# AITRICS/Medical_Tri_Modal_Pilot

Hardware: AMD Instinct MI355X
Metric: tri-modal training samples/s (fwd+bwd+AdamW step, per-GPU batch 64) (higher is better)
Workload: dtype bf16; 1 GPU; BASELINE configs[1]: vslt_img_txt tri_mbt_vsltcls, 6 layers, d_model 256, batch 64/GPU, TIE-len 1000 (N_v=1005), 224x224 CXR, 128-tok text, dropout 0.1, mbt-only-vslt 1, imgtxt-time 1; global_batch=64, parallelism=dp1

## Files before the change

### include/mtmp.h

```cpp
#ifndef MTMP_H
#define MTMP_H
#include <stdint.h>
#ifdef __cplusplus
extern "C" {
#endif

#define MTMP_F32 0
#define MTMP_BF16 1

int mtmp_abi_version(void);
const char* mtmp_last_error(void);

int mtmp_attn_fwd(int dtype, const void* q, const void* k, const void* v, void* o, const void* res, void* o_res,
                  float* lse, const int32_t* kv_len, const float* key_norms, int B, int N, int H, int ld_qkv, int ld_o,
                  float scale, void* stream);
int mtmp_attn_fwd_grouped(int dtype, int n, const void* const* q, const void* const* k, const void* const* v, void* const* o,
                          const void* const* res, void* const* o_res, float* const* lse, const int32_t* const* kv_len,
                          const int32_t* const* row_start, const float* const* key_norms, const int* N, const int* ld_qkv,
                          const int* ld_o, int B, int H, float scale, void* stream);
int mtmp_attn_bwd_grouped(int dtype, int n, const void* const* q, const void* const* k, const void* const* v,
                          const void* const* o, const void* const* d_o, const float* const* lse, const int32_t* const* kv_len,
                          const int32_t* const* row_start, void* const* dq, void* const* dk, void* const* dv,
                          float* const* delta_ws, const int* N, const int* ld_qkv, const int* ld_o, const int* ld_do,
                          const int* ld_dqkv, int B, int H, float scale, void* stream);
int mtmp_attn_cls_fwd(int dtype, const void* q, const void* k, const void* v, int ld_qkv, const void* res, int ld_res, void* o_cls,
                      void* r1_cls, float* lse, const int32_t* kv_len, const int32_t* row_start, int B, int N, int H, int cls_tok,
                      float scale, void* stream);
int mtmp_attn_cls_bwd(int dtype, const void* q, const void* k, const void* v, int ld_qkv, const void* o_cls, const void* d_o,
                      const float* lse, const int32_t* kv_len, const int32_t* row_start, void* dq, void* dk, void* dv, int ld_dqkv,
                      int B, int N, int H, int cls_tok, float scale, void* stream);
long long mtmp_key_norms_floats(long long rows, int H);
int mtmp_key_norms(int dtype, const void* k, float* out, long long rows, int H, int ld, void* stream);

int mtmp_attn_bwd(int dtype, const void* q, const void* k, const void* v, const void* o, const void* d_o,
                  const float* lse, const int32_t* kv_len, void* dq, void* dk, void* dv, float* delta_ws, int B,
                  int N, int H, int ld_qkv, int ld_o, int ld_do, int ld_dqkv, float scale, void* stream);

int mtmp_ln_gemm(int dtype, const void* x, const float* gamma, const float* beta, const void* w, const float* bias,
                 void* y, void* xn, float* stats, int M, int N, int ldx, int ldy, float eps, int relu, float drop_p,
                 unsigned seed, const unsigned* seed_dev, void* stream);

int mtmp_ln_gemm_qkv(int dtype, const void* x, const float* gamma, const float* beta, const void* w, const float* bias,
                     void* y, void* xn, float* stats, float* key_norms, int M, int ldx, float eps, void* stream);

int mtmp_gemm_nt(int dtype, const void* a, const void* w, const float* bias, const void* res, void* y, int M, int N,
                 int K, int lda, int ldy, int ldr, int act, float drop_p, unsigned seed, const unsigned* seed_dev,
                 const void* gate, float gate_scale, const float* row_scale, int rows_per_scale, void* stream);

long long mtmp_sign_bits_bytes(int M, int N);
int mtmp_ln_gemm_signs(int dtype, const void* x, const float* gamma, const float* beta, const void* w, const float* bias,
                       void* y, void* xn, float* stats, int M, int N, int ldx, int ldy, float eps, float drop_p,
                       unsigned seed, const unsigned* seed_dev, void* signs, void* stream);
int mtmp_gemm_nt_signs(int dtype, const void* a, const void* w, void* y, int M, int N, int lda, int ldy,
                       const void* signs, float gate_scale, void* stream);
int mtmp_gemm_nt_signs_drop(int dtype, const void* a, const void* w, void* y, int M, int N, int lda, int ldy,
                            const void* signs, float gate_scale, float drop_p, unsigned seed, const unsigned* seed_dev,
                            void* a_out, void* stream);

long long mtmp_gemm_tn_ws_floats(int M, int N, int K);
int mtmp_gemm_tn(int dtype, const void* dy, const void* x, float* dw, float* db, float* ws, int M, int N, int K,
                 int ldy, int ldx, void* stream);
int mtmp_gemm_tn_live(int dtype, const void* dy, const void* x, float* dw, float* db, float* ws, int M, int N, int K,
                      int ldy, int ldx, const int32_t* rows_live, void* stream);

int mtmp_dropout_bwd(int dtype, const void* g_in, void* g_out, long long n, unsigned seed, const unsigned* seed_dev,
                     float p, void* stream);

int mtmp_ln_bwd_ws_floats(int M);
int mtmp_ln_bwd(int dtype, const void* z, int ldz, const float* stats, const float* gamma, const void* dy,
                const void* d_res, int ldr, void* dz, float* dgamma_dbeta, float* ws, int M, float eps, void* stream);

int mtmp_gemm_lnbwd_ws_floats(int M);
int mtmp_gemm_lnbwd(int dtype, const void* dy, const void* wt, const void* z, int ldz, const float* stats,
                    const float* gamma, const void* d_res, int ldr, void* dz, float* dgamma_dbeta, float* ws, int M,
                    int K, int ldy, float eps, void* stream);

int mtmp_tie_embed_fwd(int dtype, const float* events, const float* params, const float* ftab, void* out, int n,
                       void* stream);
int mtmp_tie_bwd_ws_floats(int n);
int mtmp_tie_embed_bwd(int dtype, const float* events, const float* params, const void* d_out, float* grads,
                       float* ws, int n, void* stream);

int mtmp_time_embed_fwd(int dtype, const float* events, const float* params, const float* ftab, void* out, int n,
                        void* stream);
int mtmp_time_embed_bwd(int dtype, const float* events, const float* params, const void* d_out, float* grads,
                        float* ws, int n, void* stream);

int mtmp_tie_embed_packed_fwd(int dtype, const float* events, const int32_t* cu_seqlens, int B, int t_pad,
                              const float* params, const float* ftab, void* out, void* stream);
int mtmp_tie_embed_packed_bwd(int dtype, const float* events, const int32_t* cu_seqlens, int B, int t_pad,
                              const float* params, const void* d_out, float* grads, float* ws, void* stream);

int mtmp_stream_input_ws_floats(int rows);
int mtmp_stream_input_fwd(int dtype, const void* x, const float* cls, const float* gamma, const float* beta,
                          const float* pe, const float* bott, void* out, float* stats, int B, int N, int nb, float eps,
                          float p, unsigned seed, const unsigned* seed_dev, const int32_t* row_start, const int32_t* kv_len,
                          void* stream);
int mtmp_stream_input_bwd(int dtype, const void* dz, const void* x, const float* cls, const float* gamma,
                          const float* stats, void* dx, float* grads, float* ws, int B, int N, int nb, float p,
                          unsigned seed, const unsigned* seed_dev, const int32_t* row_start, const int32_t* kv_len,
                          void* stream);

int mtmp_head_ws_floats(int B);
int mtmp_head_fwd(const float* cls, const float* age, const float* gender, const void* const* params, float* out, float* ws,
                  int B, float ln_eps, float bn_eps, float momentum, int training, void* stream);
int mtmp_head_bwd(const float* d_out, const float* cls, const float* age, const float* gender, const void* const* params,
                  const float* ws_fwd, float* dcls, float* g_rows, float* dw1, float* g_feat, float* db2, float* ws_bwd, int B,
                  float ln_eps, int training, void* stream);
int mtmp_head_fwd_t(int cls_dtype, const void* cls, const float* age, const float* gender, const void* const* params, float* out,
                    float* ws, int B, float ln_eps, float bn_eps, float momentum, int training, long long* num_batches_tracked,
                    void* stream);
int mtmp_head_bwd_scatter(int cls_dtype, const float* d_out, const void* cls, const float* age, const float* gender,
                          const void* const* params, const float* ws_fwd, void* dcls, float* const* dst, float* ws_bwd, int B,
                          float ln_eps, int training, void* stream);

int mtmp_bce_logits_mean(const float* logits, const float* target, float* loss, float* dlogit, int n, void* stream);

int mtmp_timestamp(unsigned long long* slot, void* stream);

int mtmp_swin_stem_fwd(int dtype, const float* img, const float* w, const float* bias, const float* ln_w,
                       const float* ln_b, void* out, int n_img, int H, int W, void* stream);

int mtmp_layernorm_rows(int dtype, const void* x, const float* w, const float* b, void* y, long long rows, int C,
                        float eps, int merge, int H, int W, void* stream);

int mtmp_swin_ln_linear(int dtype, const void* x, const float* ln_w, const float* ln_b, const void* w, const float* bias,
                        void* y, long long M, int C, int N, float eps, void* stream);

int mtmp_swin_mlp(int dtype, const void* x, const float* ln_w, const float* ln_b, const void* w1, const float* b1,
                  const void* w2, const float* b2, const float* row_scale, int rows_per_scale, void* y, long long M, int C,
                  float eps, void* stream);

int mtmp_swin_window_attn(int dtype, const void* qkv, const void* table, void* out, int n_img, int H, int W, int C,
                          int heads, int shift, float scale, void* stream);

int mtmp_adamw_step(float* param, const float* grad, float* exp_avg, float* exp_avg_sq, void* bf16_shadow,
                    long long n, float lr, float beta1, float beta2, float eps, float weight_decay, int step,
                    float grad_scale, void* stream);

int mtmp_bottleneck_exchange_fwd(int dtype, void* z_v, void* z_i, void* z_t, int B, int n_v, int n_i, int n_t,
                                 const long long* missing, int resbottle, const float* prev, float* keep,
                                 const int32_t* row_start_v, void* stream);
int mtmp_bottleneck_exchange_bwd(int dtype, void* dz_v, void* dz_i, void* dz_t, int B, int n_v, int n_i, int n_t,
                                 const long long* missing, int resbottle, const float* d_prev_in, float* d_prev_out,
                                 const int32_t* row_start_v, void* stream);

int mtmp_ln_gemm_qkv_grouped(int dtype, int n, const void* const* x, const float* const* gamma, const float* const* beta,
                             const void* const* w, const float* const* bias, void* const* y, void* const* xn, float* const* stats,
                             float* const* key_norms, const int* M, const int* ldx, float eps, const int32_t* const* rows_live,
                             void* stream);
int mtmp_ln_gemm_signs_grouped(int dtype, int n, const void* const* x, const float* const* gamma, const float* const* beta,
                               const void* const* w, const float* const* bias, void* const* y, void* const* xn, float* const* stats,
                               void* const* signs, const int* M, int N, const int* ldx, float eps, float drop_p,
                               const unsigned* seeds, const unsigned* seed_dev, const int32_t* const* rows_live, void* stream);
int mtmp_gemm_nt_grouped(int dtype, int n, const void* const* a, const void* const* w, const float* const* bias,
                         const void* const* res, void* const* y, const int* M, int N, int K, const int* lda, const int* ldy,
                         const int* ldr, int act, float drop_p, const unsigned* seeds, const unsigned* seed_dev,
                         const int32_t* const* rows_live, void* stream);
int mtmp_gemm_nt_signs_drop_grouped(int dtype, int n, const void* const* a, const void* const* w, void* const* y, const int* M, int N,
                                    const int* lda, const void* const* signs, float gate_scale, float drop_p, const unsigned* seeds,
                                    const unsigned* seed_dev, void* const* a_out, const int32_t* const* rows_live, void* stream);
int mtmp_gemm_lnbwd_grouped(int dtype, int n, const void* const* dy, const void* const* wt, const void* const* z, const int* ldz,
                            const float* const* stats, const float* const* gamma, const void* const* d_res, const int* ldr,
                            void* const* dz, float* const* ws, const int* M, int K, const int* ldy, float eps,
                            const int32_t* const* rows_live, void* stream);
int mtmp_gemm_tn_group_plan(int n, const int* M, int N, int K, int* splits_out);
int mtmp_gemm_tn_grouped(int dtype, int n, const void* const* dy, const void* const* x, float* const* ws, const int* M, int N, int K,
                         const int* ldy, const int* ldx, const int* splits, const int32_t* const* rows_live, void* stream);

int mtmp_gemm_tn_slab_rows(int dtype, int M, int N, int K);
int mtmp_gemm_lnbwd_slab_rows(int M);
int mtmp_reduce_batch(const float* const* slab, const int* rows, const long long* cols, float* const* out_a, const long long* split,
                      float* const* out_b, int n, void* stream);

int mtmp_stream_input_slab_rows(int rows);
int mtmp_stream_input_bwd_partials(int dtype, const void* dz, const void* x, const float* cls, const float* gamma, const float* stats,
                                   void* dx, float* ws, int B, int N, int nb, float p, unsigned seed, const unsigned* seed_dev,
                                   const int32_t* row_start, const int32_t* kv_len, void* stream);
int mtmp_stream_input_bwd_grouped(int dtype, int n, const void* const* dz, const void* const* x, const float* const* cls,
                                  const float* const* gamma, const float* const* stats, void* const* dx, float* ws, const int* B,
                                  const int* N, const int* nb, const float* p, const unsigned* seed, const unsigned* seed_dev,
                                  const int32_t* const* row_start, const int32_t* const* kv_len, const void* const* add,
                                  const int* add_L, void* stream);
int mtmp_stream_input_fwd_add(int dtype, const void* x, const float* cls, const float* gamma, const float* beta, const float* pe,
                              const float* bott, void* out, float* stats, int B, int N, int nb, float eps, float p, unsigned seed,
                              const unsigned* seed_dev, const int32_t* row_start, const int32_t* kv_len, const void* add,
                              int add_L, void* stream);
int mtmp_token_sums(int dtype, int n, const void* const* dx, void* const* out, const int* rows, const int* L, void* stream);
int mtmp_tie_bwd_slab_rows(int n);
int mtmp_tie_time_embed_bwd_partials(int dtype, const float* events, int n, const float* time_events, int n_time, int n_time_a,
                                     const float* params, const void* d_out, const void* d_time_a, const void* d_time_b, float* ws,
                                     void* stream);
int mtmp_reduce_scatter(const float* const* src, const int* rows, const long long* ld, const long long* cols, float* const* out, int n,
                        void* stream);

int mtmp_publish_scalar(const float* value, unsigned* pair, void* stream);

int mtmp_copy_batch(const void* const* src, void* const* dst, const long long* bytes, const int* round16, int n, void* stream);

int mtmp_transpose_batch(int elem_bytes, const void* const* src, void* const* dst, const int* rows, const int* cols, int n,
                         void* stream);

int mtmp_stream_lengths(const long long* len_v, const long long* len_i, const long long* len_t, int* out, int B, int n_bott,
                        int txt_idx, void* stream);
int mtmp_image_slots(const long long* pattern, int present_below, int32_t* out, int B, int hw0, void* stream);
int mtmp_swin_stem_fwd_live(int dtype, const float* img, const float* w, const float* bias, const float* ln_w, const float* ln_b,
                            void* out, int n_img, int H, int W, const int32_t* order, const int32_t* rows_live, void* stream);
int mtmp_layernorm_rows_live(int dtype, const void* x, const float* w, const float* b, void* y, long long rows, int C, float eps,
                             int merge, int H, int W, const int32_t* rows_live, void* stream);
int mtmp_swin_ln_linear_live(int dtype, const void* x, const float* ln_w, const float* ln_b, const void* w, const float* bias,
                             void* y, long long M, int C, int N, float eps, const int32_t* rows_live, void* stream);
int mtmp_swin_mlp_live(int dtype, const void* x, const float* ln_w, const float* ln_b, const void* w1, const float* b1,
                       const void* w2, const float* b2, const float* row_scale, int rows_per_scale, void* y, long long M, int C,
                       float eps, const int32_t* rows_live, void* stream);
int mtmp_swin_window_attn_live(int dtype, const void* qkv, const void* table, void* out, int n_img, int H, int W, int C, int heads,
                               int shift, float scale, const int32_t* rows_live, void* stream);

int mtmp_layernorm_rows_bwd_slab_rows(long long rows, int C);
int mtmp_layernorm_rows_bwd(int dtype, const void* x, const float* w, const void* dy, void* dx, float* slab, long long rows, int C,
                            float eps, void* stream);
int mtmp_gelu_fwd(int dtype, const void* x, void* y, long long n, void* stream);
int mtmp_gelu_bwd(int dtype, const void* x, const void* dy, void* dx, long long n, void* stream);
int mtmp_swin_window_attn_bwd(int dtype, const void* qkv, const void* table, const void* dout, void* dqkv, float* dtab, int n_img,
                              int H, int W, int C, int heads, int shift, float scale, void* stream);

int mtmp_swin_attn_block(int dtype, const void* x, const float* ln_w, const float* ln_b, float eps, const void* wqkv,
                         const float* bqkv, const void* table, const void* wproj, const float* bproj, const float* row_scale,
                         void* out, int n_img, int H, int W, int C, int heads, int shift, float scale, const int32_t* rows_live,
                         void* stream);
int mtmp_gemm_nt_live(int dtype, const void* a, const void* w, const float* bias, const void* res, void* y, int M, int N, int K,
                      int lda, int ldy, int ldr, int act, float drop_p, unsigned seed, const unsigned* seed_dev, const void* gate,
                      float gate_scale, const float* row_scale, int rows_per_scale, const int32_t* rows_live, void* stream);

int mtmp_row_starts(const int32_t* kv_len, int32_t* out, int B, int n_max, void* stream);

#ifdef __cplusplus
}
#endif
#endif
```

### medical_tri_modal_pilot_amd/_lib.py

```python
import ctypes
import os
from ctypes import c_char_p, c_float, c_int, c_longlong, c_uint, c_void_p

_HERE = os.path.dirname(os.path.abspath(__file__))
LIB_PATH = os.environ.get("MTMP_LIB", os.path.join(_HERE, "libmtmp_hip.so"))

F32, BF16 = 0, 1

SIGNATURES = {
    "mtmp_abi_version": (c_int, []),
    "mtmp_last_error": (c_char_p, []),
    "mtmp_attn_fwd": (c_int, [c_int] + [c_void_p] * 9 + [c_int] * 5 + [c_float, c_void_p]),
    "mtmp_attn_cls_fwd": (c_int, [c_int] + [c_void_p] * 3 + [c_int, c_void_p, c_int] + [c_void_p] * 5 + [c_int] * 4 + [c_float, c_void_p]),
    "mtmp_attn_cls_bwd": (c_int, [c_int] + [c_void_p] * 3 + [c_int] + [c_void_p] * 8 + [c_int] * 5 + [c_float, c_void_p]),
    "mtmp_attn_fwd_grouped": (c_int, [c_int, c_int] + [c_void_p] * 13 + [c_int, c_int, c_float, c_void_p]),
    "mtmp_attn_bwd_grouped": (c_int, [c_int, c_int] + [c_void_p] * 17 + [c_int, c_int, c_float, c_void_p]),
    "mtmp_key_norms_floats": (c_longlong, [c_longlong, c_int]),
    "mtmp_key_norms": (c_int, [c_int, c_void_p, c_void_p, c_longlong, c_int, c_int, c_void_p]),
    "mtmp_attn_bwd": (c_int, [c_int] + [c_void_p] * 11 + [c_int] * 7 + [c_float, c_void_p]),
    "mtmp_ln_gemm": (c_int, [c_int] + [c_void_p] * 8 + [c_int] * 4 + [c_float, c_int, c_float, c_uint, c_void_p, c_void_p]),
    "mtmp_ln_gemm_qkv": (c_int, [c_int] + [c_void_p] * 9 + [c_int, c_int, c_float, c_void_p]),
    "mtmp_gemm_nt": (c_int, [c_int] + [c_void_p] * 5 + [c_int] * 7 + [c_float, c_uint, c_void_p, c_void_p, c_float, c_void_p, c_int,
                             c_void_p]),
    "mtmp_gemm_nt_live": (c_int, [c_int] + [c_void_p] * 5 + [c_int] * 7 + [c_float, c_uint, c_void_p, c_void_p, c_float, c_void_p, c_int,
                             c_void_p, c_void_p]),
    "mtmp_sign_bits_bytes": (c_longlong, [c_int, c_int]),
    "mtmp_ln_gemm_signs": (c_int, [c_int] + [c_void_p] * 8 + [c_int] * 4 + [c_float, c_float, c_uint, c_void_p, c_void_p, c_void_p]),
    "mtmp_gemm_nt_signs": (c_int, [c_int] + [c_void_p] * 3 + [c_int] * 4 + [c_void_p, c_float, c_void_p]),
    "mtmp_gemm_nt_signs_drop": (c_int, [c_int] + [c_void_p] * 3 + [c_int] * 4 + [c_void_p, c_float, c_float, c_uint, c_void_p,
                                                                                   c_void_p, c_void_p]),
    "mtmp_ln_gemm_qkv_grouped": (c_int, [c_int, c_int] + [c_void_p] * 11 + [c_float, c_void_p, c_void_p]),
    "mtmp_ln_gemm_signs_grouped": (c_int, [c_int, c_int] + [c_void_p] * 10 + [c_int, c_void_p, c_float, c_float, c_void_p, c_void_p,
                                                                                   c_void_p, c_void_p]),
    "mtmp_gemm_nt_grouped": (c_int, [c_int, c_int] + [c_void_p] * 6 + [c_int, c_int] + [c_void_p] * 3 + [c_int, c_float, c_void_p,
                                                                                                       c_void_p, c_void_p, c_void_p]),
    "mtmp_gemm_nt_signs_drop_grouped": (c_int, [c_int, c_int] + [c_void_p] * 4 + [c_int, c_void_p, c_void_p, c_float, c_float,
                                                                                  c_void_p, c_void_p, c_void_p, c_void_p, c_void_p]),
    "mtmp_gemm_lnbwd_grouped": (c_int, [c_int, c_int] + [c_void_p] * 11 + [c_int, c_void_p, c_float, c_void_p, c_void_p]),
    "mtmp_gemm_tn_group_plan": (c_int, [c_int, c_void_p, c_int, c_int, c_void_p]),
    "mtmp_gemm_tn_grouped": (c_int, [c_int, c_int] + [c_void_p] * 4 + [c_int, c_int] + [c_void_p] * 4 + [c_void_p]),
    "mtmp_gemm_tn_slab_rows": (c_int, [c_int] * 4),
    "mtmp_gemm_lnbwd_slab_rows": (c_int, [c_int]),
    "mtmp_reduce_batch": (c_int, [c_void_p] * 6 + [c_int, c_void_p]),
    "mtmp_reduce_scatter": (c_int, [c_void_p] * 5 + [c_int, c_void_p]),
    "mtmp_stream_input_slab_rows": (c_int, [c_int]),
    "mtmp_stream_input_bwd_partials": (c_int, [c_int] + [c_void_p] * 7 + [c_int] * 3 + [c_float, c_uint, c_void_p, c_void_p, c_void_p, c_void_p]),
    "mtmp_stream_input_bwd_grouped": (c_int, [c_int, c_int] + [c_void_p] * 18),
    "mtmp_stream_input_fwd_add": (c_int, [c_int] + [c_void_p] * 8 + [c_int] * 3 + [c_float, c_float, c_uint, c_void_p, c_void_p, c_void_p, c_void_p, c_int, c_void_p]),
    "mtmp_token_sums": (c_int, [c_int, c_int] + [c_void_p] * 5),
    "mtmp_tie_bwd_slab_rows": (c_int, [c_int]),
    "mtmp_tie_time_embed_bwd_partials": (c_int, [c_int, c_void_p, c_int, c_void_p, c_int, c_int] + [c_void_p] * 6),
    "mtmp_publish_scalar": (c_int, [c_void_p, c_void_p, c_void_p]),
    "mtmp_copy_batch": (c_int, [c_void_p] * 4 + [c_int, c_void_p]),
    "mtmp_stream_lengths": (c_int, [c_void_p] * 4 + [c_int] * 3 + [c_void_p]),
    "mtmp_row_starts": (c_int, [c_void_p, c_void_p, c_int, c_int, c_void_p]),
    "mtmp_image_slots": (c_int, [c_void_p, c_int, c_void_p, c_int, c_int, c_void_p]),
    "mtmp_transpose_batch": (c_int, [c_int, c_void_p, c_void_p, c_void_p, c_void_p, c_int, c_void_p]),
    "mtmp_layernorm_rows": (c_int, [c_int] + [c_void_p] * 4 + [c_longlong, c_int, c_float, c_int, c_int, c_int, c_void_p]),
    "mtmp_layernorm_rows_live": (c_int, [c_int] + [c_void_p] * 4 + [c_longlong, c_int, c_float, c_int, c_int, c_int, c_void_p, c_void_p]),
    "mtmp_swin_window_attn": (c_int, [c_int] + [c_void_p] * 3 + [c_int] * 6 + [c_float, c_void_p]),
    "mtmp_swin_window_attn_live": (c_int, [c_int] + [c_void_p] * 3 + [c_int] * 6 + [c_float, c_void_p, c_void_p]),
    "mtmp_layernorm_rows_bwd_slab_rows": (c_int, [c_longlong, c_int]),
    "mtmp_layernorm_rows_bwd": (c_int, [c_int] + [c_void_p] * 5 + [c_longlong, c_int, c_float, c_void_p]),
    "mtmp_gelu_fwd": (c_int, [c_int, c_void_p, c_void_p, c_longlong, c_void_p]),
    "mtmp_gelu_bwd": (c_int, [c_int, c_void_p, c_void_p, c_void_p, c_longlong, c_void_p]),
    "mtmp_swin_window_attn_bwd": (c_int, [c_int] + [c_void_p] * 5 + [c_int] * 6 + [c_float, c_void_p]),
    "mtmp_gemm_tn_ws_floats": (c_longlong, [c_int, c_int, c_int]),
    "mtmp_gemm_tn": (c_int, [c_int] + [c_void_p] * 5 + [c_int] * 5 + [c_void_p]),
    "mtmp_gemm_tn_live": (c_int, [c_int] + [c_void_p] * 5 + [c_int] * 5 + [c_void_p, c_void_p]),
    "mtmp_ln_bwd_ws_floats": (c_int, [c_int]),
    "mtmp_ln_bwd": (c_int, [c_int, c_void_p, c_int, c_void_p, c_void_p, c_void_p, c_void_p, c_int, c_void_p,
                            c_void_p, c_void_p, c_int, c_float, c_void_p]),
    "mtmp_gemm_lnbwd_ws_floats": (c_int, [c_int]),
    "mtmp_gemm_lnbwd": (c_int, [c_int, c_void_p, c_void_p, c_void_p, c_int, c_void_p, c_void_p, c_void_p, c_int, c_void_p,
                                c_void_p, c_void_p, c_int, c_int, c_int, c_float, c_void_p]),
    "mtmp_tie_embed_fwd": (c_int, [c_int] + [c_void_p] * 4 + [c_int, c_void_p]),
    "mtmp_tie_bwd_ws_floats": (c_int, [c_int]),
    "mtmp_tie_embed_bwd": (c_int, [c_int] + [c_void_p] * 5 + [c_int, c_void_p]),
    "mtmp_time_embed_fwd": (c_int, [c_int] + [c_void_p] * 4 + [c_int, c_void_p]),
    "mtmp_time_embed_bwd": (c_int, [c_int] + [c_void_p] * 5 + [c_int, c_void_p]),
    "mtmp_tie_embed_packed_fwd": (c_int, [c_int, c_void_p, c_void_p, c_int, c_int, c_void_p, c_void_p, c_void_p, c_void_p]),
    "mtmp_tie_embed_packed_bwd": (c_int, [c_int, c_void_p, c_void_p, c_int, c_int, c_void_p, c_void_p, c_void_p, c_void_p, c_void_p]),
    "mtmp_stream_input_ws_floats": (c_int, [c_int]),
    "mtmp_stream_input_fwd": (c_int, [c_int] + [c_void_p] * 8 + [c_int] * 3 + [c_float, c_float, c_uint, c_void_p, c_void_p, c_void_p, c_void_p]),
    "mtmp_stream_input_bwd": (c_int, [c_int] + [c_void_p] * 8 + [c_int] * 3 + [c_float, c_uint, c_void_p, c_void_p, c_void_p, c_void_p]),
    "mtmp_head_ws_floats": (c_int, [c_int]),
    "mtmp_head_fwd": (c_int, [c_void_p] * 6 + [c_int, c_float, c_float, c_float, c_int, c_void_p]),
    "mtmp_head_bwd": (c_int, [c_void_p] * 12 + [c_int, c_float, c_int, c_void_p]),
    "mtmp_head_fwd_t": (c_int, [c_int] + [c_void_p] * 6 + [c_int, c_float, c_float, c_float, c_int, c_void_p, c_void_p]),
    "mtmp_head_bwd_scatter": (c_int, [c_int] + [c_void_p] * 9 + [c_int, c_float, c_int, c_void_p]),
    "mtmp_bce_logits_mean": (c_int, [c_void_p] * 4 + [c_int, c_void_p]),
    "mtmp_timestamp": (c_int, [c_void_p, c_void_p]),
    "mtmp_swin_ln_linear": (c_int, [c_int] + [c_void_p] * 6 + [c_longlong, c_int, c_int, c_float, c_void_p]),
    "mtmp_swin_ln_linear_live": (c_int, [c_int] + [c_void_p] * 6 + [c_longlong, c_int, c_int, c_float, c_void_p, c_void_p]),
    "mtmp_swin_mlp": (c_int, [c_int] + [c_void_p] * 8 + [c_int, c_void_p, c_longlong, c_int, c_float, c_void_p]),
    "mtmp_swin_mlp_live": (c_int, [c_int] + [c_void_p] * 8 + [c_int, c_void_p, c_longlong, c_int, c_float, c_void_p, c_void_p]),
    "mtmp_swin_attn_block": (c_int, [c_int] + [c_void_p] * 3 + [c_float] + [c_void_p] * 7 + [c_int] * 6 + [c_float, c_void_p, c_void_p]),
    "mtmp_swin_stem_fwd": (c_int, [c_int] + [c_void_p] * 6 + [c_int] * 3 + [c_void_p]),
    "mtmp_swin_stem_fwd_live": (c_int, [c_int] + [c_void_p] * 6 + [c_int] * 3 + [c_void_p, c_void_p, c_void_p]),
    "mtmp_adamw_step": (c_int, [c_void_p] * 5 + [c_longlong] + [c_float] * 5 + [c_int, c_float, c_void_p]),
    "mtmp_bottleneck_exchange_fwd": (c_int, [c_int] + [c_void_p] * 3 + [c_int] * 4 + [c_void_p, c_int, c_void_p, c_void_p, c_void_p, c_void_p]),
    "mtmp_bottleneck_exchange_bwd": (c_int, [c_int] + [c_void_p] * 3 + [c_int] * 4 + [c_void_p, c_int, c_void_p, c_void_p, c_void_p, c_void_p]),
    "mtmp_dropout_bwd": (c_int, [c_int, c_void_p, c_void_p, c_longlong, c_uint, c_void_p, c_float, c_void_p]),
}

_lib = None


def lib():
    global _lib
    if _lib is None:
        if not os.path.exists(LIB_PATH):
            raise RuntimeError(
                f"{LIB_PATH} not found: the HIP extension is not built. Run `python -c 'import __graft_entry__ as g; "
                "g.build()'` (or `make -C medical_tri_modal_pilot_amd/csrc`). There is no CPU fallback.")
        L = ctypes.CDLL(LIB_PATH)
        for name, (res, args) in SIGNATURES.items():
            fn = getattr(L, name)
            fn.restype, fn.argtypes = res, args
        _lib = L
    return _lib


def check(rc: int, what: str = ""):
    if rc != 0:
        msg = lib().mtmp_last_error()
        raise RuntimeError(f"libmtmp_hip {what} failed (status {rc}): {msg.decode() if msg else '?'}")


def call(name: str, *args):
    check(getattr(lib(), name)(*args), name)
```

### medical_tri_modal_pilot_amd/csrc/attention.hip

```cpp
#include "common.hip.h"
#include <math.h>
#include <type_traits>

namespace {

constexpr int DH = 64;
constexpr int KT = 64;
constexpr int LDT = DH + 8;
constexpr float LOG2E = 1.4426950408889634f;

template <typename T> struct AttnArgs {
    const T* q; const T* k; const T* v;
    T* o; const T* res; T* o_res;
    float* lse; const int* kv_len;
    const float* knorm;
    int B, N, H, ld_qkv, ld_o;
    float scale;
    const int* row_start = nullptr;
};

constexpr int LDR = 96;

template <typename T> constexpr int tr_elems() { return sizeof(T) == 2 ? KT * LDR : DH * LDT; }

template <typename T> MTMP_DEV void tile_map(int tid, int& ra, int& rb, int& col) {
    if (sizeof(T) == 2) { ra = tid >> 3; rb = ra + 32; col = (tid & 7) * 8; }
    else                { ra = (tid & 31) * 2; rb = ra + 1; col = (tid >> 5) * 8; }
}
typedef short s16x4 __attribute__((ext_vector_type(4)));
MTMP_DEV Frag<bf16> frag_tr(const bf16* img, int row0, int col0, int lane) {
    const int G = lane >> 4, i = lane & 15;
    const bf16* a = img + (row0 + 8 * (G >> 1) + (i >> 2)) * LDR + col0 + 16 * (G & 1) + 4 * (i & 3);
    typedef __attribute__((address_space(3))) s16x4 lds_s16x4;
    const s16x4 lo = __builtin_amdgcn_ds_read_tr16_b64_v4i16((lds_s16x4*)a);
    const s16x4 hi = __builtin_amdgcn_ds_read_tr16_b64_v4i16((lds_s16x4*)(a + 4 * LDR));
    typedef short s16x8 __attribute__((ext_vector_type(8)));
    Frag<bf16> f;
    f.v = __builtin_bit_cast(bf16x8, s16x8{lo[0], lo[1], lo[2], lo[3], hi[0], hi[1], hi[2], hi[3]});
    return f;
}
MTMP_DEV Frag<float> frag_tr(const float* img, int row0, int col0, int lane) {
    return frag_load<float>(img + (col0 + (lane & 31)) * LDT + row0 + 8 * (lane >> 5));
}

template <typename T>
MTMP_DEV void tile_qk(f32x16& acc, const T* lds_rows, int r, int half, const Frag<T> (&bf)[4]) {
    const T* arow = lds_rows + swz23(r) * LDT + 8 * half;
    acc = mma0<T>(frag_load<T>(arow), bf[0]);
#pragma unroll
    for (int c = 1; c < 4; ++c) mma<T>(acc, frag_load<T>(arow + 16 * c), bf[c]);
}

template <typename T> struct TileR { Frag<T> a, b; };

template <typename T> MTMP_DEV void put_rows_r(T* dst, const TileR<T>& t, int tid) {
    int ra, rb, col;
    tile_map<T>(tid, ra, rb, col);
    frag_store<T>(dst + ra * LDT + col, t.a);
    frag_store<T>(dst + rb * LDT + col, t.b);
}
MTMP_DEV void put_tr_r(bf16* dst, const TileR<bf16>& t, int tid) {
    int ra, rb, col;
    tile_map<bf16>(tid, ra, rb, col);
    frag_store<bf16>(dst + ra * LDR + col, t.a);
    frag_store<bf16>(dst + rb * LDR + col, t.b);
}
MTMP_DEV void put_tr_r(float* dst, const TileR<float>& t, int tid) {
    float* d = dst + (tid >> 5) * 8 * LDT + (tid & 31) * 2;
#pragma unroll
    for (int e = 0; e < 8; ++e) *reinterpret_cast<f32x2*>(d + e * LDT) = f32x2{t.a.v[e], t.b.v[e]};
}
template <typename T> MTMP_DEV Frag<T> frag_scale(const Frag<T>& f, float s) {
    Frag<T> r;
#pragma unroll
    for (int j = 0; j < 8; ++j) r.v[j] = from_f32<T>(to_f32(f.v[j]) * s);
    return r;
}
constexpr float FAST_BOUND = 64.0f;
constexpr int FWD_QW = 64;
constexpr int FWD_QWG = 4 * FWD_QW;

template <typename T> constexpr int fwd_stage_elems() { return KT * LDT + tr_elems<T>(); }

template <typename T>
__global__ __launch_bounds__(256, (sizeof(T) == 2 ? 2 : 1)) void attn_fwd_kernel(Grouped<AttnArgs<T>> grp) {
    extern __shared__ __attribute__((aligned(16))) char smem_raw[];
    T* sbase = reinterpret_cast<T*>(smem_raw);
    const int wg = xcd_remap(blockIdx.x, gridDim.x);
    const int seg = grp_find(grp, wg);
    const AttnArgs<T>& p = grp.seg[seg];
    const int w = wg - grp.first[seg];
    const int nqt = (p.N + FWD_QWG - 1) / FWD_QWG;
    const int qt = w % nqt, bh = w / nqt, hd = bh % p.H;
    const int b = p.row_start ? p.row_start[p.B + 1 + bh / p.H] : bh / p.H;
    const int tid = threadIdx.x, lane = tid & 63, wave = tid >> 6;
    const int r = lane & 31, half = lane >> 5;
    int kvl = p.kv_len ? min(p.kv_len[b], p.N) : p.N;
    const int row0 = p.row_start ? p.row_start[b] : b * p.N;
    const int Nq = p.row_start ? max(kvl, 0) : p.N;
    if (qt * FWD_QWG >= Nq) return;
    const bool uniform = kvl <= 0;
    if (uniform) kvl = Nq;
    const size_t base = (size_t)row0 * p.ld_qkv + hd * DH;
    const T* Qb = p.q + base; const T* Kb = p.k + base; const T* Vb = p.v + base;
    const int q0w = qt * FWD_QWG + wave * FWD_QW;
    const int blk0 = row0 >> 5, blk1 = (row0 + Nq - 1) >> 5;
    float km = 0.f;
    if (p.knorm) km = p.knorm[(size_t)min(blk0 + lane, blk1) * p.H + hd];
    Frag<T> qf[2][4];
#pragma unroll
    for (int qb = 0; qb < 2; ++qb) {
        const int qrow = q0w + 32 * qb + r;
#pragma unroll
        for (int c = 0; c < 4; ++c)
            qf[qb][c] = frag_keep(frag_load<T>(Qb + (size_t)min(qrow, Nq - 1) * p.ld_qkv + 16 * c + 8 * half),
                                  qrow < Nq && !uniform);
    }
    const float c2 = p.scale * LOG2E;
    f32x16 o[2][2] = {{{0}, {0}}, {{0}, {0}}};
    float m[2] = {-INFINITY, -INFINITY}, l[2] = {0.f, 0.f};
    const int nfull = kvl / KT, ntiles = (kvl + KT - 1) / KT;
    int ra, rb, col;
    tile_map<T>(tid, ra, rb, col);
    const size_t tstep = (size_t)KT * p.ld_qkv;
    const T* kpa = Kb + (size_t)ra * p.ld_qkv + col;
    const T* kpb = Kb + (size_t)rb * p.ld_qkv + col;
    const ptrdiff_t kv_off = Vb - Kb;
    TileR<T> kreg, vreg;
    auto fetch = [&](int t) {
        if (t < nfull) {
            kreg.a = frag_load<T>(kpa); kreg.b = frag_load<T>(kpb);
            vreg.a = frag_load<T>(kpa + kv_off); vreg.b = frag_load<T>(kpb + kv_off);
            kpa += tstep; kpb += tstep;
        } else {
            const T* ka = Kb + (size_t)min(t * KT + ra, kvl - 1) * p.ld_qkv + col;
            const T* kb_ = Kb + (size_t)min(t * KT + rb, kvl - 1) * p.ld_qkv + col;
            kreg.a = frag_load<T>(ka); kreg.b = frag_load<T>(kb_);
            vreg.a = frag_load<T>(ka + kv_off); vreg.b = frag_load<T>(kb_ + kv_off);
        }
    };
    auto put = [&](int t) {
        T* sK = sbase + (t & 1) * fwd_stage_elems<T>();
        put_rows_r<T>(sK, kreg, tid);
        put_tr_r(sK + KT * LDT, vreg, tid);
    };
    fetch(0);
    bool fast = false;
    if (p.knorm) {
        float qs = 0.f;
#pragma unroll
        for (int qb = 0; qb < 2; ++qb) {
            float s = 0.f;
#pragma unroll
            for (int c = 0; c < 4; ++c)
#pragma unroll
                for (int j = 0; j < 8; ++j) s = fmaf(to_f32(qf[qb][c].v[j]), to_f32(qf[qb][c].v[j]), s);
            qs = fmaxf(qs, s);
        }
        qs = half_sum(qs) ;
        for (int i = blk0 + lane + 64; i <= blk1; i += 64) km = fmaxf(km, p.knorm[(size_t)i * p.H + hd]);
        km = wave_max(km);
        const float bound = sqrtf(qs) * km * (c2 * 1.02f);
        fast = wave_all(bound <= FAST_BOUND);
    }
    put(0);
    if (ntiles > 1) fetch(1);
    auto tile_begin = [&](int it) {
        __syncthreads();
        if (it + 1 < ntiles) put(it + 1);
        if (it + 2 < ntiles) fetch(it + 2);
    };
    auto load_k = [&](const T* sK, int kb, Frag<T> (&ka)[4]) {
        const T* arow = sK + (32 * kb + swz23(r)) * LDT + 8 * half;
#pragma unroll
        for (int c = 0; c < 4; ++c) ka[c] = frag_load<T>(arow + 16 * c);
    };
    auto load_v = [&](const T* sV, int kb, Frag<T> (&vt)[2][2]) {
#pragma unroll
        for (int s = 0; s < 2; ++s) {
            vt[s][0] = frag_tr(sV, 32 * kb + 16 * s, 0, lane);
            vt[s][1] = frag_tr(sV, 32 * kb + 16 * s, 32, lane);
        }
    };
    auto scores = [&](f32x16& st, const Frag<T> (&ka)[4], int qb) {
        st = mma0<T>(ka[0], qf[qb][0]);
#pragma unroll
        for (int c = 1; c < 4; ++c) mma<T>(st, ka[c], qf[qb][c]);
    };
    auto tail_c = [&](int k0) {
        f32x16 c;
#pragma unroll
        for (int t = 0; t < 16; ++t) c[t] = (k0 + acc_row_swz(t, half) >= kvl) ? -INFINITY : 0.f;
        return c;
    };
    auto scores_c = [&](f32x16& st, const Frag<T> (&ka)[4], int qb, const f32x16& c) {
        st = mma_c<T>(ka[0], qf[qb][0], c);
#pragma unroll
        for (int c4 = 1; c4 < 4; ++c4) mma<T>(st, ka[c4], qf[qb][c4]);
    };
    auto pv = [&](int qb, const Frag<T> (&pf)[2], const Frag<T> (&vt)[2][2]) {
#pragma unroll
        for (int s = 0; s < 2; ++s) {
            mma<T>(o[qb][0], vt[s][0], pf[s]);
            mma<T>(o[qb][1], vt[s][1], pf[s]);
        }
    };
    if (fast) {
#pragma unroll
        for (int qb = 0; qb < 2; ++qb)
#pragma unroll
            for (int c = 0; c < 4; ++c) qf[qb][c] = frag_scale<T>(qf[qb][c], c2);
        auto soft = [&](f32x16& st, int qb, Frag<T> (&pf)[2]) {
#pragma unroll
            for (int t = 0; t < 16; ++t) {
                const float e = fast_exp2(st[t]);
                l[qb] += e;
                st[t] = e;
            }
            pf[0] = frag_from_acc<T>(st, 0);
            pf[1] = frag_from_acc<T>(st, 1);
        };
        auto interleave = [&]() {
            if (sizeof(T) == 2) {
#pragma unroll
                for (int g = 0; g < 4; ++g) {
                    __builtin_amdgcn_sched_group_barrier(0x008, 1, 0);
                    __builtin_amdgcn_sched_group_barrier(0x400, 4, 0);
                }
#pragma unroll
                for (int g = 0; g < 4; ++g) {
                    __builtin_amdgcn_sched_group_barrier(0x008, 1, 0);
                    __builtin_amdgcn_sched_group_barrier(0x002, 6, 0);
                }
            }
        };
        auto body_rot = [&](int it, auto tail_tag, f32x16& s11, Frag<T> (&p01)[2], Frag<T> (&vtp)[2][2]) {
            constexpr bool TAIL = decltype(tail_tag)::value;
            __syncthreads();
            const T* sK = sbase + (it & 1) * fwd_stage_elems<T>();
            const T* sV = sK + KT * LDT;
            const int k0 = it * KT;
            f32x16 s00, s10, s01;
            Frag<T> ka0[4], ka1[4], vt0[2][2], p00[2], p10[2], p11[2];
            load_k(sK, 0, ka0);
            if (it + 1 < ntiles) put(it + 1);
            if (it + 2 < ntiles) fetch(it + 2);
            f32x16 c0, c1;
            if (TAIL) { c0 = tail_c(k0); c1 = tail_c(k0 + 32); }
            pv(0, p01, vtp);
            if (TAIL) scores_c(s00, ka0, 0, c0); else scores(s00, ka0, 0);
            soft(s11, 1, p11);
            load_v(sV, 0, vt0);
            interleave();
            __builtin_amdgcn_sched_barrier(0);
            pv(1, p11, vtp);
            if (TAIL) scores_c(s10, ka0, 1, c0); else scores(s10, ka0, 1);
            soft(s00, 0, p00);
            load_k(sK, 1, ka1);
            interleave();
            __builtin_amdgcn_sched_barrier(0);
            pv(0, p00, vt0);
            if (TAIL) scores_c(s01, ka1, 0, c1); else scores(s01, ka1, 0);
            soft(s10, 1, p10);
            load_v(sV, 1, vtp);
            interleave();
            __builtin_amdgcn_sched_barrier(0);
            pv(1, p10, vt0);
            if (TAIL) scores_c(s11, ka1, 1, c1); else scores(s11, ka1, 1);
            soft(s01, 0, p01);
            interleave();
            __builtin_amdgcn_sched_barrier(0);
        };
        {
            f32x16 s11;
            Frag<T> p01[2] = {frag_zero<T>(), frag_zero<T>()}, vtp[2][2] = {{frag_zero<T>(), frag_zero<T>()}, {frag_zero<T>(), frag_zero<T>()}};
#pragma unroll
            for (int t = 0; t < 16; ++t) s11[t] = -INFINITY;
            for (int it = 0; it < nfull; ++it) body_rot(it, std::false_type{}, s11, p01, vtp);
            if (ntiles > nfull) body_rot(nfull, std::true_type{}, s11, p01, vtp);
            Frag<T> p11[2];
            pv(0, p01, vtp);
            soft(s11, 1, p11);
            __builtin_amdgcn_sched_barrier(0);
            pv(1, p11, vtp);
        }
        m[0] = m[1] = 0.f;
    } else {
        auto body = [&](int it, auto tail_tag) {
            constexpr bool TAIL = decltype(tail_tag)::value;
            tile_begin(it);
            const T* sK = sbase + (it & 1) * fwd_stage_elems<T>();
            const T* sV = sK + KT * LDT;
#pragma unroll
            for (int kb = 0; kb < 2; ++kb) {
                Frag<T> ka[4], vt[2][2];
                load_k(sK, kb, ka);
                load_v(sV, kb, vt);
                f32x16 ct;
                if (TAIL) ct = tail_c(it * KT + 32 * kb);
#pragma unroll
                for (int qb = 0; qb < 2; ++qb) {
                    f32x16 st;
                    if (TAIL) scores_c(st, ka, qb, ct); else scores(st, ka, qb);
                    const float seed = fmaxf(st[15], st[14]);
                    float mxa = max3(seed, st[0], st[1]), mxb = max3(seed, st[2], st[3]);
#pragma unroll
                    for (int t = 4; t < 12; t += 4) {
                        mxa = max3(mxa, st[t], st[t + 1]);
                        mxb = max3(mxb, st[t + 2], st[t + 3]);
                    }
                    const float mx = half_max(max3(mxa, mxb, fmaxf(st[12], st[13]))) * c2;
                    if (!wave_all(mx <= m[qb])) {
                        const float m_new = fmaxf(m[qb], mx);
                        const float alpha = fast_exp2(m[qb] - m_new);
                        l[qb] *= alpha; o[qb][0] *= alpha; o[qb][1] *= alpha;
                        m[qb] = m_new;
                    }
#pragma unroll
                    for (int t = 0; t < 16; ++t) {
                        const float e = fast_exp2(fmaf(st[t], c2, -m[qb]));
                        l[qb] += e;
                        st[t] = e;
                    }
                    Frag<T> pf[2] = {frag_from_acc<T>(st, 0), frag_from_acc<T>(st, 1)};
                    pv(qb, pf, vt);
                }
            }
        };
        for (int it = 0; it < nfull; ++it) body(it, std::false_type{});
        if (ntiles > nfull) body(nfull, std::true_type{});
    }
    constexpr int E = 16 / (int)sizeof(T);
    constexpr int CH = DH * (int)sizeof(T) / 16, RPP = 64 / CH, NPS = FWD_QW / RPP;
    const int rsub = lane / CH, ch = lane % CH;
    u32x4_t rv[NPS];
    if (p.o_res) {
#pragma unroll
        for (int ps = 0; ps < NPS; ++ps) {
            const int rowc = min(q0w + ps * RPP + rsub, Nq - 1);
            rv[ps] = *reinterpret_cast<const u32x4_t*>(p.res + ((size_t)row0 + rowc) * p.ld_o + hd * DH + ch * E);
        }
    }
    __syncthreads();
    T* sO = reinterpret_cast<T*>(smem_raw) + wave * FWD_QW * LDT;
#pragma unroll
    for (int qb = 0; qb < 2; ++qb) {
        l[qb] = half_sum(l[qb]);
        const float inv = 1.0f / l[qb];
#pragma unroll
        for (int dt = 0; dt < 2; ++dt)
#pragma unroll
            for (int g = 0; g < 4; ++g) {
                const f32x16& ov = o[qb][dt];
                store4<T>(sO + (32 * qb + r) * LDT + 32 * dt + 8 * g + 4 * half, ov[4 * g] * inv, ov[4 * g + 1] * inv,
                          ov[4 * g + 2] * inv, ov[4 * g + 3] * inv);
            }
        const int qrow = q0w + 32 * qb + r;
        if (qrow < Nq && half == 0) p.lse[((size_t)b * p.H + hd) * p.N + qrow] = m[qb] + log2f(l[qb]);
    }
    asm volatile("s_waitcnt lgkmcnt(0)" ::: "memory");
    u32x4_t ovv[NPS];
#pragma unroll
    for (int ps = 0; ps < NPS; ++ps)
        ovv[ps] = *reinterpret_cast<const u32x4_t*>(reinterpret_cast<const char*>(sO + (ps * RPP + rsub) * LDT) + 16 * ch);
    T* orow = p.o + ((size_t)row0 + q0w + rsub) * p.ld_o + hd * DH + ch * E;
#pragma unroll
    for (int ps = 0; ps < NPS; ++ps)
        if (q0w + ps * RPP + rsub < Nq) *reinterpret_cast<u32x4_t*>(orow + (size_t)ps * RPP * p.ld_o) = ovv[ps];
    if (p.o_res) {
        T* rrow = p.o_res + ((size_t)row0 + q0w + rsub) * p.ld_o + hd * DH + ch * E;
#pragma unroll
        for (int ps = 0; ps < NPS; ++ps) {
            T ob[E], rbv[E], sb[E];
            __builtin_memcpy(ob, &ovv[ps], 16);
            __builtin_memcpy(rbv, &rv[ps], 16);
#pragma unroll
            for (int i = 0; i < E; ++i) sb[i] = from_f32<T>(to_f32(ob[i]) + to_f32(rbv[i]));
            u32x4_t sv;
            __builtin_memcpy(&sv, sb, 16);
            if (q0w + ps * RPP + rsub < Nq) *reinterpret_cast<u32x4_t*>(rrow + (size_t)ps * RPP * p.ld_o) = sv;
        }
    }
}

template <typename T> __global__ __launch_bounds__(256) void key_norms_kernel(const T* k, float* out, int M, int H, int ld) {
    const int lane = threadIdx.x & 63, blk = blockIdx.x * 4 + (threadIdx.x >> 6);
    if (blk * 32 >= M) return;
    const int rsub = lane >> 3, ch = lane & 7;
    for (int h = 0; h < H; ++h) {
        float best = 0.f;
#pragma unroll
        for (int ps = 0; ps < 4; ++ps) {
            const int row = min(blk * 32 + ps * 8 + rsub, M - 1);
            const Frag<T> f = frag_load<T>(k + (size_t)row * ld + h * DH + 8 * ch);
            float s = 0.f;
#pragma unroll
            for (int j = 0; j < 8; ++j) s = fmaf(to_f32(f.v[j]), to_f32(f.v[j]), s);
            s += __shfl_xor(s, 1, 64); s += __shfl_xor(s, 2, 64); s += __shfl_xor(s, 4, 64);
            best = fmaxf(best, s);
        }
        best = fmaxf(best, __shfl_xor(best, 8, 64));
        best = fmaxf(best, __shfl_xor(best, 16, 64));
        best = fmaxf(best, __shfl_xor(best, 32, 64));
        if (lane == 0) out[(size_t)blk * H + h] = sqrtf(best);
    }
}



template <typename T> struct DualTile;
template <> struct DualTile<bf16> {
    static constexpr int BYTES = 8192;
    static MTMP_DEV void map(int tid, int& ra, int& rb, int& ca, int& cb) { ra = rb = tid >> 2; ca = 8 * (tid & 3); cb = 32 + 8 * (tid & 3); }
    static MTMP_DEV int off(int row, int ch) {
        return 1024 * (row >> 3) + 512 * (ch >> 2) + 64 * (row & 7) + 16 * ((ch & 3) ^ ((row >> 2) & 3));
    }
    static MTMP_DEV void put(char* img, const TileR<bf16>& t, int tid) {
        const int row = tid >> 2, c = tid & 3;
        *reinterpret_cast<bf16x8*>(img + off(row, c)) = t.a.v;
        *reinterpret_cast<bf16x8*>(img + off(row, 4 + c)) = t.b.v;
    }
    static MTMP_DEV Frag<bf16> row_frag(const char* img, int row, int c, int half) {
        Frag<bf16> f;
        f.v = *reinterpret_cast<const bf16x8*>(img + off(row, 2 * c + half));
        return f;
    }
    static MTMP_DEV Frag<bf16> tr_frag(const char* img, int row0, int col0, int lane) {
        const int G = lane >> 4, i = lane & 15;
        const int row = row0 + 8 * (G >> 1) + (i >> 2), col = col0 + 16 * (G & 1) + 4 * (i & 3);
        typedef __attribute__((address_space(3))) s16x4 lds_s16x4;
        const s16x4 lo = __builtin_amdgcn_ds_read_tr16_b64_v4i16((lds_s16x4*)(img + off(row, col >> 3) + 2 * (col & 7)));
        const s16x4 hi = __builtin_amdgcn_ds_read_tr16_b64_v4i16((lds_s16x4*)(img + off(row + 4, col >> 3) + 2 * (col & 7)));
        typedef short s16x8 __attribute__((ext_vector_type(8)));
        Frag<bf16> f;
        f.v = __builtin_bit_cast(bf16x8, s16x8{lo[0], lo[1], lo[2], lo[3], hi[0], hi[1], hi[2], hi[3]});
        return f;
    }
};
template <> struct DualTile<float> {
    static constexpr int BYTES = (KT * LDT + DH * LDT) * 4;
    static MTMP_DEV void map(int tid, int& ra, int& rb, int& ca, int& cb) { ra = (tid & 31) * 2; rb = ra + 1; ca = cb = (tid >> 5) * 8; }
    static MTMP_DEV void put(char* img, const TileR<float>& t, int tid) {
        float* rows = reinterpret_cast<float*>(img);
        put_rows_r<float>(rows, t, tid);
        put_tr_r(rows + KT * LDT, t, tid);
    }
    static MTMP_DEV Frag<float> row_frag(const char* img, int row, int c, int half) {
        return frag_load<float>(reinterpret_cast<const float*>(img) + row * LDT + 16 * c + 8 * half);
    }
    static MTMP_DEV Frag<float> tr_frag(const char* img, int row0, int col0, int lane) {
        return frag_tr(reinterpret_cast<const float*>(img) + KT * LDT, row0, col0, lane);
    }
};

template <typename T> struct TileStream {
    const T* base; const T* pa; const T* pb;
    size_t step; int ld, limit, ra, rb, ca, cb, nfull;
    MTMP_DEV void init(const T* src, int ld_, int limit_, int tid) {
        DualTile<T>::map(tid, ra, rb, ca, cb);
        base = src; ld = ld_; limit = limit_; nfull = limit_ / KT; step = (size_t)KT * ld_;
        pa = src + (size_t)ra * ld_ + ca; pb = src + (size_t)rb * ld_ + cb;
    }
    MTMP_DEV TileR<T> fetch(int t) {
        TileR<T> x;
        if (t < nfull) {
            x.a = frag_load<T>(pa); x.b = frag_load<T>(pb);
            pa += step; pb += step;
        } else {
            x.a = frag_load<T>(base + (size_t)min(t * KT + ra, limit - 1) * ld + ca);
            x.b = frag_load<T>(base + (size_t)min(t * KT + rb, limit - 1) * ld + cb);
        }
        return x;
    }
    MTMP_DEV TileR<T> zero_tail(const TileR<T>& x, int t) const {
        TileR<T> y;
        y.a = frag_keep(x.a, t * KT + ra < limit);
        y.b = frag_keep(x.b, t * KT + rb < limit);
        return y;
    }
};
template <typename T> struct AttnBwdArgs {
    const T* q; const T* k; const T* v; const T* d_o;
    const float* lse; float* delta; const int* kv_len;
    T* dq; T* dk; T* dv;
    int B, N, H, ld_qkv, ld_do, ld_dqkv;
    float scale;
    const T* o; int ld_o;
    const int* row_start = nullptr;
};


template <typename T> constexpr int dq_stage_bytes() { return 2 * DualTile<T>::BYTES; }
template <typename T>
__global__ __launch_bounds__(256, (sizeof(T) == 2 ? 2 : 1)) void attn_bwd_dq_kernel(Grouped<AttnBwdArgs<T>> grp) {
    using DT = DualTile<T>;
    extern __shared__ __attribute__((aligned(16))) char smem_raw[];
    const int wg = xcd_remap(blockIdx.x, gridDim.x);
    const int seg = grp_find(grp, wg);
    const AttnBwdArgs<T>& p = grp.seg[seg];
    const int w = wg - grp.first[seg];
    const int nqt = (p.N + 127) >> 7;
    const int qt = w % nqt, bh = w / nqt, hd = bh % p.H;
    const int b = p.row_start ? p.row_start[p.B + 1 + bh / p.H] : bh / p.H;
    const int tid = threadIdx.x, lane = tid & 63, wave = tid >> 6;
    const int r = lane & 31, half = lane >> 5;
    int kvl = p.kv_len ? min(p.kv_len[b], p.N) : p.N;
    const int row0 = p.row_start ? p.row_start[b] : b * p.N;
    const int Nq = p.row_start ? max(kvl, 0) : p.N;
    if (qt * 128 >= Nq) return;
    const bool uniform = kvl <= 0;
    if (uniform) kvl = Nq;
    const size_t base = (size_t)row0 * p.ld_qkv + hd * DH;
    const T* Qb = p.q + base; const T* Kb = p.k + base; const T* Vb = p.v + base;
    const int qrow = qt * 128 + wave * 32 + r;
    const float c2 = p.scale * LOG2E;
    const size_t sidx = ((size_t)b * p.H + hd) * p.N + min(qrow, Nq - 1);
    const float lse_v = p.lse[sidx];
    Frag<T> qf[4], dof[4], of[4];
#pragma unroll
    for (int c = 0; c < 4; ++c) {
        qf[c] = frag_load<T>(Qb + (size_t)min(qrow, Nq - 1) * p.ld_qkv + 16 * c + 8 * half);
        dof[c] = frag_load<T>(p.d_o + ((size_t)row0 + min(qrow, Nq - 1)) * p.ld_do + hd * DH + 16 * c + 8 * half);
        of[c] = frag_load<T>(p.o + ((size_t)row0 + min(qrow, Nq - 1)) * p.ld_o + hd * DH + 16 * c + 8 * half);
    }
    const int ntiles = uniform ? 0 : (kvl + KT - 1) / KT;
    const int nfull = kvl / KT;
    TileStream<T> ks, vs;
    ks.init(Kb, p.ld_qkv, kvl, tid);
    vs.init(Vb, p.ld_qkv, kvl, tid);
    TileR<T> kreg, vreg;
    auto fetch = [&](int t) { kreg = ks.fetch(t); vreg = vs.fetch(t); };
    auto put = [&](int t) {
        char* st_ = smem_raw + (t & 1) * dq_stage_bytes<T>();
        DT::put(st_, t >= nfull ? ks.zero_tail(kreg, t) : kreg, tid);
        DT::put(st_ + DT::BYTES, vreg, tid);
    };
    if (ntiles > 0) fetch(0);
#pragma unroll
    for (int c = 0; c < 4; ++c) {
        qf[c] = frag_keep(frag_scale<T>(qf[c], c2), qrow < Nq);
        dof[c] = frag_keep(dof[c], qrow < Nq);
    }
    float dsum = 0.f;
#pragma unroll
    for (int c = 0; c < 4; ++c)
#pragma unroll
        for (int jx = 0; jx < 8; ++jx) dsum = fmaf(to_f32(dof[c].v[jx]), to_f32(of[c].v[jx]), dsum);
    dsum = half_sum(dsum);
    if (qrow < Nq && half == 0) p.delta[sidx] = dsum;
    const float nL = (qrow < Nq) ? -lse_v : -INFINITY;
    const float nD = (qrow < Nq) ? -dsum : 0.f;
    f32x16 cL, cD;
#pragma unroll
    for (int t = 0; t < 16; ++t) { cL[t] = nL; cD[t] = nD; }
    f32x16 dq0 = {0}, dq1 = {0};
    if (ntiles > 0) put(0);
    if (ntiles > 1) fetch(1);
    struct Unit { f32x16 st, dp; };
    auto body = [&](int it, auto tail_tag) {
        constexpr bool TAIL = decltype(tail_tag)::value;
        const int k0 = it * KT;
        __syncthreads();
        const char* sK = smem_raw + (it & 1) * dq_stage_bytes<T>();
        const char* sV = sK + DT::BYTES;
        auto load_rows = [&](int kb, Frag<T> (&ka)[4], Frag<T> (&va)[4]) {
            const int row = 32 * kb + swz23(r);
#pragma unroll
            for (int c = 0; c < 4; ++c) { ka[c] = DT::row_frag(sK, row, c, half); va[c] = DT::row_frag(sV, row, c, half); }
        };
        auto load_tr = [&](int kb, Frag<T> (&trf)[2][2]) {
#pragma unroll
            for (int s = 0; s < 2; ++s) {
                trf[s][0] = DT::tr_frag(sK, 32 * kb + 16 * s, 0, lane);
                trf[s][1] = DT::tr_frag(sK, 32 * kb + 16 * s, 32, lane);
            }
        };
        auto scores = [&](int kb, Unit& u, const Frag<T> (&ka)[4], const Frag<T> (&va)[4]) {
            if (TAIL) {
                f32x16 cLt;
#pragma unroll
                for (int t = 0; t < 16; ++t) cLt[t] = (k0 + 32 * kb + acc_row_swz(t, half) < kvl) ? nL : -INFINITY;
                u.st = mma_c<T>(ka[0], qf[0], cLt);
            } else
            u.st = mma_c<T>(ka[0], qf[0], cL);
#pragma unroll
            for (int c = 1; c < 4; ++c) mma<T>(u.st, ka[c], qf[c]);
            u.dp = mma_c<T>(va[0], dof[0], cD);
#pragma unroll
            for (int c = 1; c < 4; ++c) mma<T>(u.dp, va[c], dof[c]);
        };
        auto soft = [&](Unit& u, Frag<T> (&dsf)[2]) {
#pragma unroll
            for (int t = 0; t < 16; ++t) u.st[t] = fast_exp2(u.st[t]) * u.dp[t];
            dsf[0] = frag_from_acc<T>(u.st, 0);
            dsf[1] = frag_from_acc<T>(u.st, 1);
        };
        auto grad = [&](const Frag<T> (&dsf)[2], const Frag<T> (&trf)[2][2]) {
#pragma unroll
            for (int s = 0; s < 2; ++s) {
                mma<T>(dq0, trf[s][0], dsf[s]);
                mma<T>(dq1, trf[s][1], dsf[s]);
            }
        };
        Unit u0, u1;
        Frag<T> d0[2], d1[2], ka0[4], va0[4], ka1[4], va1[4], tr0[2][2], tr1[2][2];
        load_rows(0, ka0, va0);
        if (it + 1 < ntiles) put(it + 1);
        if (it + 2 < ntiles) fetch(it + 2);
        __builtin_amdgcn_sched_barrier(0);
        load_rows(1, ka1, va1);
        scores(0, u0, ka0, va0);
        if (sizeof(T) == 2) {
#pragma unroll
            for (int g = 0; g < 8; ++g) {
                __builtin_amdgcn_sched_group_barrier(0x008, 1, 0);
                __builtin_amdgcn_sched_group_barrier(0x100, 1, 0);
            }
        }
        __builtin_amdgcn_sched_barrier(0);
        load_tr(0, tr0);
        scores(1, u1, ka1, va1);
        soft(u0, d0);
        if (sizeof(T) == 2) {
#pragma unroll
            for (int g = 0; g < 8; ++g) {
                __builtin_amdgcn_sched_group_barrier(0x008, 1, 0);
                __builtin_amdgcn_sched_group_barrier(0x100, 1, 0);
                __builtin_amdgcn_sched_group_barrier(0x400, 2, 0);
                __builtin_amdgcn_sched_group_barrier(0x002, 3, 0);
            }
        }
        __builtin_amdgcn_sched_barrier(0);
        load_tr(1, tr1);
        grad(d0, tr0);
        soft(u1, d1);
        if (sizeof(T) == 2) {
#pragma unroll
            for (int g = 0; g < 4; ++g) {
                __builtin_amdgcn_sched_group_barrier(0x008, 1, 0);
                __builtin_amdgcn_sched_group_barrier(0x100, 2, 0);
                __builtin_amdgcn_sched_group_barrier(0x400, 4, 0);
                __builtin_amdgcn_sched_group_barrier(0x002, 6, 0);
            }
        }
        __builtin_amdgcn_sched_barrier(0);
        grad(d1, tr1);
    };
    for (int it = 0; it < min(nfull, ntiles); ++it) body(it, std::false_type{});
    if (ntiles > nfull) body(nfull, std::true_type{});
    if (qrow < Nq) {
        const size_t orow = ((size_t)row0 + qrow) * p.ld_dqkv + hd * DH;
#pragma unroll
        for (int dt = 0; dt < 2; ++dt)
#pragma unroll
            for (int g = 0; g < 4; ++g) {
                const f32x16& o = dt ? dq1 : dq0;
                const int d0 = 32 * dt + 8 * g + 4 * half;
                store4<T>(p.dq + orow + d0, o[4 * g] * p.scale, o[4 * g + 1] * p.scale, o[4 * g + 2] * p.scale,
                          o[4 * g + 3] * p.scale);
            }
    }
}

template <typename T> constexpr int dkdv_stage_bytes() { return 2 * DualTile<T>::BYTES + 2 * KT * (int)sizeof(float); }
template <typename T>
__global__ __launch_bounds__(256, (sizeof(T) == 2 ? 2 : 1)) void attn_bwd_dkdv_kernel(Grouped<AttnBwdArgs<T>> grp) {
    using DT = DualTile<T>;
    extern __shared__ __attribute__((aligned(16))) char smem_raw[];
    const int wg = xcd_remap(blockIdx.x, gridDim.x);
    const int seg = grp_find(grp, wg);
    const AttnBwdArgs<T>& p = grp.seg[seg];
    const int w = wg - grp.first[seg];
    const int nkt = (p.N + 127) >> 7;
    const int kt = w % nkt, bh = w / nkt, hd = bh % p.H;
    const int b = p.row_start ? p.row_start[p.B + 1 + bh / p.H] : bh / p.H;
    const int tid = threadIdx.x, lane = tid & 63, wave = tid >> 6;
    const int r = lane & 31, half = lane >> 5;
    int kvl = p.kv_len ? min(p.kv_len[b], p.N) : p.N;
    const int row0 = p.row_start ? p.row_start[b] : b * p.N;
    const int Nq = p.row_start ? max(kvl, 0) : p.N;
    if (kt * 128 >= Nq) return;
    const bool uniform = kvl <= 0;
    if (uniform) kvl = Nq;
    const size_t base = (size_t)row0 * p.ld_qkv + hd * DH;
    const T* Qb = p.q + base; const T* Kb = p.k + base; const T* Vb = p.v + base;
    const T* dOb = p.d_o + (size_t)row0 * p.ld_do + hd * DH;
    const float* Lb = p.lse + ((size_t)b * p.H + hd) * p.N;
    const float* Db = p.delta + ((size_t)b * p.H + hd) * p.N;
    const int kw0 = kt * 128 + wave * 32;
    const int key = kw0 + r;
    f32x16 dk0 = {0}, dk1 = {0}, dv0 = {0}, dv1 = {0};
    if (kt * 128 < kvl) {
        const float c2 = p.scale * LOG2E;
        Frag<T> kf[4], vf[4];
#pragma unroll
        for (int c = 0; c < 4; ++c) {
            kf[c] = frag_keep(frag_scale<T>(frag_load<T>(Kb + (size_t)min(key, kvl - 1) * p.ld_qkv + 16 * c + 8 * half), c2),
                              key < kvl && !uniform);
            vf[c] = frag_keep(frag_load<T>(Vb + (size_t)min(key, kvl - 1) * p.ld_qkv + 16 * c + 8 * half), key < kvl);
        }
        const int nq = (Nq + KT - 1) / KT;
        TileStream<T> qs, os;
        qs.init(Qb, p.ld_qkv, Nq, tid);
        os.init(dOb, p.ld_do, Nq, tid);
        TileR<T> qreg, oreg;
        const int lrow = tid & (KT - 1);
        float lreg, dreg;
        auto fetch = [&](int t) {
            qreg = qs.fetch(t);
            oreg = os.fetch(t);
            const int qn = min(t * KT + lrow, Nq - 1);
            lreg = Lb[qn];
            dreg = Db[qn];
        };
        auto put = [&](int t) {
            char* st_ = smem_raw + (t & 1) * dkdv_stage_bytes<T>();
            DT::put(st_, qreg, tid);
            DT::put(st_ + DT::BYTES, oreg, tid);
            if (tid < KT) {
                float* sL = reinterpret_cast<float*>(st_ + 2 * DT::BYTES);
                sL[tid] = (t * KT + tid < Nq) ? -lreg : -INFINITY;
                sL[KT + tid] = (t * KT + tid < Nq) ? -dreg : 0.f;
            }
        };
        fetch(0);
        put(0);
        if (nq > 1) fetch(1);
        for (int it = 0; it < nq; ++it) {
            __syncthreads();
            if (it + 1 < nq) put(it + 1);
            if (it + 2 < nq) fetch(it + 2);
            if (kw0 < kvl) {
                const char* sQ = smem_raw + (it & 1) * dkdv_stage_bytes<T>();
                const char* sdO = sQ + DT::BYTES;
                const float* sL = reinterpret_cast<const float*>(sQ + 2 * DT::BYTES);
                const float* sD = sL + KT;
                auto load_rowconst = [&](int qb, f32x16& cL, f32x16& cD) {
#pragma unroll
                    for (int h8 = 0; h8 < 2; ++h8)
#pragma unroll
                        for (int v = 0; v < 2; ++v) {
                            const f32x4 l4 = *reinterpret_cast<const f32x4*>(sL + 32 * qb + 16 * h8 + 8 * half + 4 * v);
                            const f32x4 d4 = *reinterpret_cast<const f32x4*>(sD + 32 * qb + 16 * h8 + 8 * half + 4 * v);
#pragma unroll
                            for (int i = 0; i < 4; ++i) { cL[8 * h8 + 4 * v + i] = l4[i]; cD[8 * h8 + 4 * v + i] = d4[i]; }
                        }
                };
                auto load_rows = [&](int qb, Frag<T> (&qa)[4], Frag<T> (&oa)[4]) {
                    const int row = 32 * qb + swz23(r);
#pragma unroll
                    for (int c = 0; c < 4; ++c) { qa[c] = DT::row_frag(sQ, row, c, half); oa[c] = DT::row_frag(sdO, row, c, half); }
                };
                auto load_tr = [&](int qb, Frag<T> (&trf)[2][4]) {
#pragma unroll
                    for (int s = 0; s < 2; ++s) {
                        const int q16 = 32 * qb + 16 * s;
                        trf[s][0] = DT::tr_frag(sdO, q16, 0, lane);
                        trf[s][1] = DT::tr_frag(sdO, q16, 32, lane);
                        trf[s][2] = DT::tr_frag(sQ, q16, 0, lane);
                        trf[s][3] = DT::tr_frag(sQ, q16, 32, lane);
                    }
                };
                auto scores = [&](f32x16& st, f32x16& ds, const f32x16& cL, const f32x16& cD, const Frag<T> (&qa)[4],
                                  const Frag<T> (&oa)[4]) {
                    st = mma_c<T>(qa[0], kf[0], cL);
#pragma unroll
                    for (int c = 1; c < 4; ++c) mma<T>(st, qa[c], kf[c]);
                    ds = mma_c<T>(oa[0], vf[0], cD);
#pragma unroll
                    for (int c = 1; c < 4; ++c) mma<T>(ds, oa[c], vf[c]);
                };
                auto probs = [&](f32x16& st, f32x16& ds, Frag<T> (&pf)[2], Frag<T> (&dsf)[2]) {
#pragma unroll
                    for (int t = 0; t < 16; ++t) {
                        const float pv = fast_exp2(st[t]);
                        st[t] = pv;
                        ds[t] *= pv;
                    }
#pragma unroll
                    for (int s = 0; s < 2; ++s) { pf[s] = frag_from_acc<T>(st, s); dsf[s] = frag_from_acc<T>(ds, s); }
                };
                auto grads = [&](const Frag<T> (&pf)[2], const Frag<T> (&dsf)[2], const Frag<T> (&trf)[2][4]) {
#pragma unroll
                    for (int s = 0; s < 2; ++s) {
                        mma<T>(dv0, trf[s][0], pf[s]);
                        mma<T>(dv1, trf[s][1], pf[s]);
                        mma<T>(dk0, trf[s][2], dsf[s]);
                        mma<T>(dk1, trf[s][3], dsf[s]);
                    }
                };
                f32x16 st0, ds0, st1, ds1, cL1, cD1;
                Frag<T> qa1[4], oa1[4], pf0[2], dsf0[2], pf1[2], dsf1[2];
                {
                    f32x16 cL0, cD0;
                    Frag<T> qa0[4], oa0[4];
                    load_rowconst(0, cL0, cD0);
                    load_rows(0, qa0, oa0);
                    load_rowconst(1, cL1, cD1);
                    load_rows(1, qa1, oa1);
                    scores(st0, ds0, cL0, cD0, qa0, oa0);
                }
                __builtin_amdgcn_sched_barrier(0);
                {
                    scores(st1, ds1, cL1, cD1, qa1, oa1);
                    probs(st0, ds0, pf0, dsf0);
                    if (sizeof(T) == 2) {
#pragma unroll
                        for (int g = 0; g < 8; ++g) {
                            __builtin_amdgcn_sched_group_barrier(0x008, 1, 0);
                            __builtin_amdgcn_sched_group_barrier(0x400, 2, 0);
                            __builtin_amdgcn_sched_group_barrier(0x002, 4, 0);
                        }
                    }
                }
                __builtin_amdgcn_sched_barrier(0);
                {
                    Frag<T> trf0[2][4];
                    load_tr(0, trf0);
                    grads(pf0, dsf0, trf0);
                    probs(st1, ds1, pf1, dsf1);
                    if (sizeof(T) == 2) {
                        __builtin_amdgcn_sched_group_barrier(0x100, 16, 0);
                        __builtin_amdgcn_sched_group_barrier(0x400, 4, 0);
                        __builtin_amdgcn_sched_group_barrier(0x002, 8, 0);
#pragma unroll
                        for (int g = 0; g < 8; ++g) {
                            __builtin_amdgcn_sched_group_barrier(0x008, 1, 0);
                            if (g < 6) __builtin_amdgcn_sched_group_barrier(0x400, 2, 0);
                            if (g < 6) __builtin_amdgcn_sched_group_barrier(0x002, 4, 0);
                        }
                    }
                }
                __builtin_amdgcn_sched_barrier(0);
                {
                    Frag<T> trf1[2][4];
                    load_tr(1, trf1);
                    grads(pf1, dsf1, trf1);
                }
            }
        }
    }
    if (key < Nq) {
        const bool live = key < kvl;
        const float ks = (live && !uniform) ? p.scale : 0.f, vs_ = live ? 1.f : 0.f;
        const size_t orow = ((size_t)row0 + key) * p.ld_dqkv + hd * DH;
#pragma unroll
        for (int dt = 0; dt < 2; ++dt)
#pragma unroll
            for (int g = 0; g < 4; ++g) {
                const f32x16& ak = dt ? dk1 : dk0;
                const f32x16& av = dt ? dv1 : dv0;
                const int d0 = 32 * dt + 8 * g + 4 * half;
                store4<T>(p.dk + orow + d0, ks != 0.f ? ak[4 * g] * ks : 0.f, ks != 0.f ? ak[4 * g + 1] * ks : 0.f,
                          ks != 0.f ? ak[4 * g + 2] * ks : 0.f, ks != 0.f ? ak[4 * g + 3] * ks : 0.f);
                store4<T>(p.dv + orow + d0, vs_ != 0.f ? av[4 * g] : 0.f, vs_ != 0.f ? av[4 * g + 1] : 0.f,
                          vs_ != 0.f ? av[4 * g + 2] : 0.f, vs_ != 0.f ? av[4 * g + 3] : 0.f);
            }
    }
}

#define MTMP_MFMA_FIRST(d, a, b, c) asm volatile("v_mfma_f32_32x32x16_bf16 %0, %1, %2, %3" : "=&v"(d) : "v"(a), "a"(b), "v"(c))
#define MTMP_MFMA_NEXT(d, a, b) asm volatile("v_mfma_f32_32x32x16_bf16 %0, %1, %2, %0" : "+v"(d) : "v"(a), "a"(b))
#define MTMP_MFMA_ACC(acc, a, b) asm volatile("v_mfma_f32_32x32x16_bf16 %0, %1, %2, %0" : "+a"(acc) : "v"(a), "v"(b))

#ifdef MTMP_LAB_CLOCK
__device__ long long mtmp_dbg_stamps[64 * 4 * 160];
#define STAMP(k) do { if (wg < 64 && lane == 0 && (k) < 160) mtmp_dbg_stamps[(wg * 4 + wave) * 160 + (k)] = __builtin_amdgcn_s_memtime(); } while (0)
#else
#define STAMP(k) do {} while (0)
#endif
constexpr int DKV64_KEYS = 256;
constexpr int BWD64_MIN_ROWS = 1536;
constexpr int BWD64_STAGES = 3;
constexpr int DKV64_OUT_BYTES = 2 * 64 * LDT * 2;

MTMP_DEV bf16x8 to_agpr(bf16x8 x) {
    bf16x8 y;
    asm volatile("" : "=a"(y) : "0"(x));
    return y;
}
struct PackedUnit { u32x4_t p[2], d[2]; };
MTMP_DEV unsigned cvt_pk_bf16(float lo, float hi) {
    return __builtin_bit_cast(unsigned, __builtin_convertvector(f32x2{lo, hi}, bf16x2));
}

__global__ __launch_bounds__(256, 1) void attn_bwd_dkdv64_kernel(Grouped<AttnBwdArgs<bf16>> grp) {
    using T = bf16;
    using DT = DualTile<T>;
    extern __shared__ __attribute__((aligned(16))) char smem_raw[];
    const int wg = xcd_remap(blockIdx.x, gridDim.x);
    const int seg = grp_find(grp, wg);
    const AttnBwdArgs<T>& p = grp.seg[seg];
    const int w = wg - grp.first[seg];
    const int nkt = (p.N + DKV64_KEYS - 1) / DKV64_KEYS;
    const int kt = w % nkt, bh = w / nkt, hd = bh % p.H;
    const int b = p.row_start ? p.row_start[p.B + 1 + bh / p.H] : bh / p.H;
    const int tid = threadIdx.x, lane = tid & 63, wave = tid >> 6;
    const int r = lane & 31, half = lane >> 5;
    int kvl = p.kv_len ? min(p.kv_len[b], p.N) : p.N;
    const int row0 = p.row_start ? p.row_start[b] : b * p.N;
    const int Nq = p.row_start ? max(kvl, 0) : p.N;
    if (kt * DKV64_KEYS >= Nq) return;
    STAMP(0);
    const bool uniform = kvl <= 0;
    if (uniform) kvl = Nq;
    const size_t base = (size_t)row0 * p.ld_qkv + hd * DH;
    const T* Qb = p.q + base; const T* Kb = p.k + base; const T* Vb = p.v + base;
    const T* dOb = p.d_o + (size_t)row0 * p.ld_do + hd * DH;
    const float* Lb = p.lse + ((size_t)b * p.H + hd) * p.N;
    const float* Db = p.delta + ((size_t)b * p.H + hd) * p.N;
    const int kw0 = kt * DKV64_KEYS + wave * 64;
    f32x16 dv00 = {0}, dv01 = {0}, dk00 = {0}, dk01 = {0}, dv10 = {0}, dv11 = {0}, dk10 = {0}, dk11 = {0};
    if (kt * DKV64_KEYS < kvl) {
        const float c2 = p.scale * LOG2E;
        Frag<T> kx[2][4], vx[2][4];
#pragma unroll
        for (int kb = 0; kb < 2; ++kb)
#pragma unroll
            for (int c = 0; c < 4; ++c) {
                const int key = kw0 + 32 * kb + r;
                kx[kb][c] = frag_load<T>(Kb + (size_t)min(key, kvl - 1) * p.ld_qkv + 16 * c + 8 * half);
                vx[kb][c] = frag_load<T>(Vb + (size_t)min(key, kvl - 1) * p.ld_qkv + 16 * c + 8 * half);
            }
        const int nq = (Nq + KT - 1) / KT;
        TileStream<T> qs, os;
        qs.init(Qb, p.ld_qkv, Nq, tid);
        os.init(dOb, p.ld_do, Nq, tid);
        TileR<T> qreg, oreg;
        const int lrow = tid & (KT - 1);
        float lreg, dreg;
        auto stage = [&](int t) { return smem_raw + (t % BWD64_STAGES) * dkdv_stage_bytes<T>(); };
        auto stage_piece = [&](int k, int tp, int tf) {
            if (k < 3) {
                if (tp >= nq) return;
                char* st_ = stage(tp);
                if (k == 0) DT::put(st_, qreg, tid);
                else if (k == 1) DT::put(st_ + DT::BYTES, oreg, tid);
                else if (tid < KT) {
                    float* sL = reinterpret_cast<float*>(st_ + 2 * DT::BYTES);
                    sL[tid] = (tp * KT + tid < Nq) ? -lreg : -INFINITY;
                    sL[KT + tid] = (tp * KT + tid < Nq) ? -dreg : 0.f;
                }
            } else {
                if (tf >= nq) return;
                if (k == 3) qreg = qs.fetch(tf);
                else if (k == 4) oreg = os.fetch(tf);
                else {
                    const int qn = min(tf * KT + lrow, Nq - 1);
                    lreg = Lb[qn];
                    dreg = Db[qn];
                }
            }
        };
        auto stage_all = [&](int tp, int tf) {
#pragma unroll
            for (int k = 0; k < 6; ++k) stage_piece(k, tp, tf);
        };
        stage_all(nq, 0);
        bf16x8 kf[2][4], vf[2][4];
#pragma unroll
        for (int kb = 0; kb < 2; ++kb)
#pragma unroll
            for (int c = 0; c < 4; ++c) {
                const bool live = kw0 + 32 * kb + r < kvl;
                kf[kb][c] = to_agpr(frag_keep(frag_scale<T>(kx[kb][c], c2), live && !uniform).v);
                vf[kb][c] = to_agpr(frag_keep(vx[kb][c], live).v);
            }
        stage_all(0, 1);
        __syncthreads();
        const bool active = kw0 < kvl;
        bf16x8 qa[4], oa[4], tr[2][4];
        f32x16 cL, cD;
        struct LaneOffs { unsigned rowE, rowO, cst, trA, trB; };
        LaneOffs lo;
        {
            const int sr = swz23(r), G = lane >> 4, i16 = lane & 15;
            lo.rowE = DT::off(sr, half);
            lo.rowO = DT::off(sr, 2 + half);
            lo.cst = 2 * DT::BYTES + 32 * half;
            const int trow = 8 * (G >> 1) + (i16 >> 2), tch = 2 * (G & 1) + ((i16 & 3) >> 1);
            lo.trA = DT::off(trow, tch) + 8 * (i16 & 1);
            lo.trB = DT::off(trow + 4, tch) + 8 * (i16 & 1);
            const unsigned lds0 = (unsigned)(size_t)(__attribute__((address_space(3))) char*)smem_raw;
            lo.rowE += lds0; lo.rowO += lds0; lo.cst += lds0; lo.trA += lds0; lo.trB += lds0;
        }
        typedef __attribute__((address_space(3))) const char lds_cchar;
        auto lds_at = [](unsigned ofs) { return (lds_cchar*)(size_t)ofs; };
        auto bases = [&](int t) {
            const unsigned sb = (unsigned)((t % BWD64_STAGES) * dkdv_stage_bytes<T>());
            LaneOffs x{lo.rowE + sb, lo.rowO + sb, lo.cst + sb, lo.trA + sb, lo.trB + sb};
            asm volatile("" : "+v"(x.rowE), "+v"(x.rowO), "+v"(x.cst), "+v"(x.trA), "+v"(x.trB));
            return x;
        };
        auto load_rows = [&](const LaneOffs& bs, int qb, int c, bool dO) {
            typedef __attribute__((address_space(3))) const bf16x8 lds_bf16x8;
            const bf16x8 v = *(lds_bf16x8*)(lds_at((c & 1) ? bs.rowO : bs.rowE) + 512 * (c >> 1) + 4096 * qb + (dO ? DT::BYTES : 0));
            if (dO) oa[c] = v; else qa[c] = v;
        };
        auto load_const = [&](const LaneOffs& bs, int qb, int k4, bool dlt) {
            typedef __attribute__((address_space(3))) const f32x4 lds_f32x4;
            const f32x4 v4 = *(lds_f32x4*)(lds_at(bs.cst) + (dlt ? 4 * KT : 0) + 4 * (32 * qb + 16 * (k4 >> 1) + 4 * (k4 & 1)));
#pragma unroll
            for (int i = 0; i < 4; ++i) { if (dlt) cD[4 * k4 + i] = v4[i]; else cL[4 * k4 + i] = v4[i]; }
        };
        auto load_tr = [&](const LaneOffs& bs, int qb, int s2, int j) {
            typedef __attribute__((address_space(3))) s16x4 lds_s16x4;
            const int imm = 4096 * qb + 2048 * s2 + 512 * (j & 1) + (j < 2 ? DT::BYTES : 0);
            const s16x4 a = __builtin_amdgcn_ds_read_tr16_b64_v4i16((lds_s16x4*)(lds_at(bs.trA) + imm));
            const s16x4 b4 = __builtin_amdgcn_ds_read_tr16_b64_v4i16((lds_s16x4*)(lds_at(bs.trB) + imm));
            typedef short s16x8 __attribute__((ext_vector_type(8)));
            tr[s2][j] = __builtin_bit_cast(bf16x8, s16x8{a[0], a[1], a[2], a[3], b4[0], b4[1], b4[2], b4[3]});
        };
        auto slot = [&](auto mode_tag, f32x16& sN, f32x16& dN, const bf16x8 (&kfb)[4], const bf16x8 (&vfb)[4], f32x16& sC, f32x16& dC,
                        PackedUnit& out, const PackedUnit& in, f32x16& dv0, f32x16& dv1, f32x16& dk0, f32x16& dk1,
                        const LaneOffs& st_rows, int qb_rows, const LaneOffs& st_tr, int qb_tr, int tp, int tf) {
            constexpr int MODE = decltype(mode_tag)::value;
#pragma unroll
            for (int i = 0; i < 16; ++i) {
                if (i == 0) MTMP_MFMA_FIRST(sN, qa[0], kfb[0], cL);
                else if (i < 4) MTMP_MFMA_NEXT(sN, qa[i], kfb[i]);
                else if (i == 4) MTMP_MFMA_FIRST(dN, oa[0], vfb[0], cD);
                else if (i < 8) MTMP_MFMA_NEXT(dN, oa[i - 4], vfb[i - 4]);
                else {
                    const int s2 = (i - 8) >> 2, j = (i - 8) & 3;
                    if (j == 0) MTMP_MFMA_ACC(dv0, tr[s2][0], in.p[s2]);
                    else if (j == 1) MTMP_MFMA_ACC(dv1, tr[s2][1], in.p[s2]);
                    else if (j == 2) MTMP_MFMA_ACC(dk0, tr[s2][2], in.d[s2]);
                    else MTMP_MFMA_ACC(dk1, tr[s2][3], in.d[s2]);
                }
                const float e = fast_exp2(sC[i]);
                if (i > 0) dC[i - 1] *= sC[i - 1];
                sC[i] = e;
                if (i & 1) out.p[i >> 3][(i & 7) >> 1] = cvt_pk_bf16(sC[i - 1], e);
                if (i >= 2 && !(i & 1)) out.d[(i - 2) >> 3][((i - 2) & 7) >> 1] = cvt_pk_bf16(dC[i - 2], dC[i - 1]);
                if (i == 15) {
                    dC[15] *= e;
                    out.d[1][3] = cvt_pk_bf16(dC[14], dC[15]);
                }
                if (MODE == 1) {
                    if (i < 4) load_rows(st_rows, qb_rows, i, false);
                    else if (i < 8) load_rows(st_rows, qb_rows, i - 4, true);
                    else load_tr(st_tr, qb_tr, (i - 8) >> 2, (i - 8) & 3);
                    if (i >= 1 && i < 5) load_const(st_rows, qb_rows, i - 1, false);
                    else if (i >= 5 && i < 9) load_const(st_rows, qb_rows, i - 5, true);
                }
                if (MODE == 2 && (i & 1) && i < 12) stage_piece(i >> 1, tp, tf);
                __builtin_amdgcn_sched_barrier(0);
            }
        };
        f32x16 sA, dA, sB, dB;
        PackedUnit fX, fY;
#pragma unroll
        for (int t = 0; t < 16; ++t) { sB[t] = -INFINITY; dB[t] = 0.f; }
#pragma unroll
        for (int s2 = 0; s2 < 2; ++s2) {
            fX.p[s2] = u32x4_t{0, 0, 0, 0}; fX.d[s2] = u32x4_t{0, 0, 0, 0};
#pragma unroll
            for (int j = 0; j < 4; ++j) tr[s2][j] = frag_zero<T>().v;
        }
        if (active) {
            const LaneOffs b0 = bases(0);
#pragma unroll
            for (int c = 0; c < 4; ++c) {
                load_rows(b0, 0, c, false); load_rows(b0, 0, c, true);
                load_const(b0, 0, c, false); load_const(b0, 0, c, true);
            }
        }
        const std::integral_constant<int, 0> plain{};
        const std::integral_constant<int, 1> loads{};
        const std::integral_constant<int, 2> staging{};
        STAMP(1);
        for (int it = 0; it < nq; ++it) {
            STAMP(2 + 8 * it);
            const LaneOffs cur = bases(it);
            const LaneOffs nxt = bases(it + 1 < nq ? it + 1 : it);
            if (active) {
                __builtin_amdgcn_sched_barrier(0);
                STAMP(3 + 8 * it);
                slot(staging, sA, dA, kf[0], vf[0], sB, dB, fY, fX, dv00, dv01, dk00, dk01, cur, 0, cur, 0, it + 1, it + 2);
                STAMP(4 + 8 * it);
                slot(loads, sB, dB, kf[1], vf[1], sA, dA, fX, fY, dv10, dv11, dk10, dk11, cur, 1, cur, 0, 0, 0);
                STAMP(5 + 8 * it);
                slot(plain, sA, dA, kf[0], vf[0], sB, dB, fY, fX, dv00, dv01, dk00, dk01, cur, 0, cur, 0, 0, 0);
                STAMP(6 + 8 * it);
            } else {
                stage_all(it + 1, it + 2);
            }
            __syncthreads();
            if (active) {
                STAMP(7 + 8 * it);
                slot(loads, sB, dB, kf[1], vf[1], sA, dA, fX, fY, dv10, dv11, dk10, dk11, nxt, 0, cur, 1, 0, 0);
                STAMP(8 + 8 * it);
            }
        }
        if (active) {
#pragma unroll
            for (int i = 0; i < 16; ++i) {
                if (i < 8) {
                    const int s2 = i >> 2, j = i & 3;
                    if (j == 0) MTMP_MFMA_ACC(dv00, tr[s2][0], fX.p[s2]);
                    else if (j == 1) MTMP_MFMA_ACC(dv01, tr[s2][1], fX.p[s2]);
                    else if (j == 2) MTMP_MFMA_ACC(dk00, tr[s2][2], fX.d[s2]);
                    else MTMP_MFMA_ACC(dk01, tr[s2][3], fX.d[s2]);
                }
                const float e = fast_exp2(sB[i]);
                dB[i] *= e;
                sB[i] = e;
                if (i & 1) {
                    fY.p[i >> 3][(i & 7) >> 1] = cvt_pk_bf16(sB[i - 1], e);
                    fY.d[i >> 3][(i & 7) >> 1] = cvt_pk_bf16(dB[i - 1], dB[i]);
                }
                __builtin_amdgcn_sched_barrier(0);
            }
#pragma unroll
            for (int s2 = 0; s2 < 2; ++s2) {
                MTMP_MFMA_ACC(dv10, tr[s2][0], fY.p[s2]);
                MTMP_MFMA_ACC(dv11, tr[s2][1], fY.p[s2]);
                MTMP_MFMA_ACC(dk10, tr[s2][2], fY.d[s2]);
                MTMP_MFMA_ACC(dk11, tr[s2][3], fY.d[s2]);
            }
        }
        STAMP(150);
        asm volatile("s_nop 15\n\ts_nop 15" : "+a"(dv00), "+a"(dv01), "+a"(dk00), "+a"(dk01), "+a"(dv10), "+a"(dv11), "+a"(dk10), "+a"(dk11));
    }
    T* sOut = reinterpret_cast<T*>(smem_raw + BWD64_STAGES * dkdv_stage_bytes<T>() + wave * DKV64_OUT_BYTES);
#pragma unroll
    for (int kb = 0; kb < 2; ++kb) {
        const int key = kw0 + 32 * kb + r;
        const bool live = key < kvl;
        const bool wk = live && !uniform;
#pragma unroll
        for (int dt = 0; dt < 2; ++dt)
#pragma unroll
            for (int g = 0; g < 4; ++g) {
                const f32x16& ak = kb ? (dt ? dk11 : dk10) : (dt ? dk01 : dk00);
                const f32x16& av = kb ? (dt ? dv11 : dv10) : (dt ? dv01 : dv00);
                const int d0 = 32 * dt + 8 * g + 4 * half;
                store4<T>(sOut + (32 * kb + r) * LDT + d0, wk ? ak[4 * g] * p.scale : 0.f, wk ? ak[4 * g + 1] * p.scale : 0.f,
                          wk ? ak[4 * g + 2] * p.scale : 0.f, wk ? ak[4 * g + 3] * p.scale : 0.f);
                store4<T>(sOut + (64 + 32 * kb + r) * LDT + d0, live ? av[4 * g] : 0.f, live ? av[4 * g + 1] : 0.f,
                          live ? av[4 * g + 2] : 0.f, live ? av[4 * g + 3] : 0.f);
            }
    }
    asm volatile("s_waitcnt lgkmcnt(0)" ::: "memory");
    {
        const int rsub = lane >> 3, ch = lane & 7;
        u32x4_t ok[8], ov[8];
#pragma unroll
        for (int ps = 0; ps < 8; ++ps) {
            ok[ps] = *reinterpret_cast<const u32x4_t*>(reinterpret_cast<const char*>(sOut + (8 * ps + rsub) * LDT) + 16 * ch);
            ov[ps] = *reinterpret_cast<const u32x4_t*>(reinterpret_cast<const char*>(sOut + (64 + 8 * ps + rsub) * LDT) + 16 * ch);
        }
        T* krow = p.dk + ((size_t)row0 + kw0 + rsub) * p.ld_dqkv + hd * DH + 8 * ch;
        T* vrow = p.dv + ((size_t)row0 + kw0 + rsub) * p.ld_dqkv + hd * DH + 8 * ch;
#pragma unroll
        for (int ps = 0; ps < 8; ++ps)
            if (kw0 + 8 * ps + rsub < Nq) {
                *reinterpret_cast<u32x4_t*>(krow + (size_t)8 * ps * p.ld_dqkv) = ok[ps];
                *reinterpret_cast<u32x4_t*>(vrow + (size_t)8 * ps * p.ld_dqkv) = ov[ps];
            }
    }
    STAMP(151);
}

template <typename T> size_t fwd_smem() { return (size_t)2 * fwd_stage_elems<T>() * sizeof(T); }
template <typename T> size_t dq_smem() { return (size_t)2 * dq_stage_bytes<T>(); }
template <typename T> size_t dkdv_smem() { return (size_t)2 * dkdv_stage_bytes<T>(); }

template <typename K> int set_smem(K kern, size_t bytes) {
    if (bytes > 48 * 1024) {
        if (hipFuncSetAttribute(reinterpret_cast<const void*>(kern), hipFuncAttributeMaxDynamicSharedMemorySize,
                                (int)bytes) != hipSuccess) {
            mtmp_set_error("hipFuncSetAttribute(MaxDynamicSharedMemorySize=%zu) failed", bytes);
            return MTMP_ERR_LAUNCH;
        }
    }
    return MTMP_OK;
}

template <typename A, typename F> Grouped<A> make_group(int n, const A* segs, F blocks_of, int& total) {
    Grouped<A> g;
    total = 0;
    for (int i = 0; i < GRP_MAX; ++i) {
        g.seg[i] = segs[i < n ? i : 0];
        g.first[i] = total;
        if (i < n) total += blocks_of(segs[i]);
    }
    g.first[GRP_MAX] = total;
    return g;
}

template <typename T> int launch_fwd(int n, const AttnArgs<T>* segs, hipStream_t st) {
    int nwg;
    const Grouped<AttnArgs<T>> g = make_group(n, segs, [](const AttnArgs<T>& a) { return ((a.N + FWD_QWG - 1) / FWD_QWG) * a.H * a.B; }, nwg);
    const size_t sm = fwd_smem<T>();
    if (int e = set_smem(attn_fwd_kernel<T>, sm)) return e;
    hipLaunchKernelGGL(attn_fwd_kernel<T>, dim3(nwg), dim3(256), sm, st, g);
    MTMP_CHECK_LAUNCH("mtmp_attn_fwd");
    return MTMP_OK;
}

template <typename T> int launch_bwd(int n, const AttnBwdArgs<T>* segs, hipStream_t st) {
    int nwg;
    const Grouped<AttnBwdArgs<T>> g = make_group(n, segs, [](const AttnBwdArgs<T>& a) { return ((a.N + 127) / 128) * a.H * a.B; }, nwg);
    if (int e = set_smem(attn_bwd_dq_kernel<T>, dq_smem<T>())) return e;
    hipLaunchKernelGGL(attn_bwd_dq_kernel<T>, dim3(nwg), dim3(256), dq_smem<T>(), st, g);
    MTMP_CHECK_LAUNCH("mtmp_attn_bwd(dq)");
    if constexpr (sizeof(T) == 2) {
        int nmax = 0;
        for (int i = 0; i < n; ++i) nmax = segs[i].N > nmax ? segs[i].N : nmax;
        if (nmax >= BWD64_MIN_ROWS) {
            int nwg64;
            const Grouped<AttnBwdArgs<T>> g64 =
                make_group(n, segs, [](const AttnBwdArgs<T>& a) { return ((a.N + DKV64_KEYS - 1) / DKV64_KEYS) * a.H * a.B; }, nwg64);
            const size_t sm64 = (size_t)BWD64_STAGES * dkdv_stage_bytes<T>() + 4 * DKV64_OUT_BYTES;
            if (int e = set_smem(attn_bwd_dkdv64_kernel, sm64)) return e;
            hipLaunchKernelGGL(attn_bwd_dkdv64_kernel, dim3(nwg64), dim3(256), sm64, st, g64);
            MTMP_CHECK_LAUNCH("mtmp_attn_bwd(dkdv64)");
            return MTMP_OK;
        }
    }
    if (int e = set_smem(attn_bwd_dkdv_kernel<T>, dkdv_smem<T>())) return e;
    hipLaunchKernelGGL(attn_bwd_dkdv_kernel<T>, dim3(nwg), dim3(256), dkdv_smem<T>(), st, g);
    MTMP_CHECK_LAUNCH("mtmp_attn_bwd(dkdv)");
    return MTMP_OK;
}

bool attn_shape_ok(int B, int N, int H, int ld_a, int ld_b) {
    return B > 0 && N > 0 && H > 0 && H <= 4 && ld_a >= H * DH && ld_b >= H * DH && (ld_a % 8) == 0 && (ld_b % 8) == 0;
}

}

template <typename T>
int fwd_entry(int n, const void* const* q, const void* const* k, const void* const* v, void* const* o, const void* const* res,
              void* const* o_res, float* const* lse, const int32_t* const* kv_len, const int32_t* const* row_start,
              const float* const* key_norms, const int* N, const int* ld_qkv, const int* ld_o, int B, int H, float scale,
              hipStream_t st) {
    AttnArgs<T> a[GRP_MAX];
    for (int i = 0; i < n; ++i)
        a[i] = AttnArgs<T>{(const T*)q[i], (const T*)k[i], (const T*)v[i], (T*)o[i], res ? (const T*)res[i] : nullptr,
                           o_res ? (T*)o_res[i] : nullptr, lse[i], kv_len ? kv_len[i] : nullptr, key_norms ? key_norms[i] : nullptr,
                           B, N[i], H, ld_qkv[i], ld_o[i], scale, row_start ? row_start[i] : nullptr};
    return launch_fwd<T>(n, a, st);
}

extern "C" int mtmp_attn_fwd_grouped(int dtype, int n, const void* const* q, const void* const* k, const void* const* v,
                                     void* const* o, const void* const* res, void* const* o_res, float* const* lse,
                                     const int32_t* const* kv_len, const int32_t* const* row_start, const float* const* key_norms,
                                     const int* N, const int* ld_qkv, const int* ld_o, int B, int H, float scale, void* stream) {
    MTMP_CHECK_ARG(n >= 1 && n <= GRP_MAX && q && k && v && o && lse && N && ld_qkv && ld_o, "mtmp_attn_fwd: bad group (n=%d)", n);
    for (int i = 0; i < n; ++i) {
        MTMP_CHECK_ARG(q[i] && k[i] && v[i] && o[i] && lse[i], "mtmp_attn_fwd: null pointer (stream %d)", i);
        MTMP_CHECK_ARG((!res || !res[i]) == (!o_res || !o_res[i]), "mtmp_attn_fwd: res and o_res must be given together");
        MTMP_CHECK_ARG(!(row_start && row_start[i]) || (kv_len && kv_len[i]), "mtmp_attn_fwd: a packed stream needs kv_len");
        MTMP_CHECK_ARG(attn_shape_ok(B, N[i], H, ld_qkv[i], ld_o[i]), "mtmp_attn_fwd: bad shape B=%d N=%d H=%d ld=%d/%d", B, N[i], H,
                       ld_qkv[i], ld_o[i]);
    }
    hipStream_t st = (hipStream_t)stream;
    if (dtype == 0) return fwd_entry<float>(n, q, k, v, o, res, o_res, lse, kv_len, row_start, key_norms, N, ld_qkv, ld_o, B, H, scale, st);
    if (dtype == 1) return fwd_entry<bf16>(n, q, k, v, o, res, o_res, lse, kv_len, row_start, key_norms, N, ld_qkv, ld_o, B, H, scale, st);
    mtmp_set_error("mtmp_attn_fwd: unknown dtype %d", dtype);
    return MTMP_ERR_ARG;
}

extern "C" int mtmp_attn_fwd(int dtype, const void* q, const void* k, const void* v, void* o, const void* res,
                             void* o_res, float* lse, const int32_t* kv_len, const float* key_norms, int B, int N, int H,
                             int ld_qkv, int ld_o, float scale, void* stream) {
    return mtmp_attn_fwd_grouped(dtype, 1, &q, &k, &v, &o, &res, &o_res, &lse, &kv_len, nullptr, &key_norms, &N, &ld_qkv, &ld_o, B, H,
                                 scale, stream);
}

template <typename T>
int bwd_entry(int n, const void* const* q, const void* const* k, const void* const* v, const void* const* o, const void* const* d_o,
              const float* const* lse, const int32_t* const* kv_len, const int32_t* const* row_start, void* const* dq,
              void* const* dk, void* const* dv, float* const* delta_ws, const int* N, const int* ld_qkv, const int* ld_o,
              const int* ld_do, const int* ld_dqkv, int B, int H, float scale, hipStream_t st) {
    AttnBwdArgs<T> a[GRP_MAX];
    for (int i = 0; i < n; ++i)
        a[i] = AttnBwdArgs<T>{(const T*)q[i], (const T*)k[i], (const T*)v[i], (const T*)d_o[i], lse[i], delta_ws[i],
                              kv_len ? kv_len[i] : nullptr, (T*)dq[i], (T*)dk[i], (T*)dv[i], B, N[i], H, ld_qkv[i], ld_do[i],
                              ld_dqkv[i], scale, (const T*)o[i], ld_o[i], row_start ? row_start[i] : nullptr};
    return launch_bwd<T>(n, a, st);
}

extern "C" int mtmp_attn_bwd_grouped(int dtype, int n, const void* const* q, const void* const* k, const void* const* v,
                                     const void* const* o, const void* const* d_o, const float* const* lse,
                                     const int32_t* const* kv_len, const int32_t* const* row_start, void* const* dq,
                                     void* const* dk, void* const* dv, float* const* delta_ws, const int* N, const int* ld_qkv,
                                     const int* ld_o, const int* ld_do, const int* ld_dqkv, int B, int H, float scale, void* stream) {
    MTMP_CHECK_ARG(n >= 1 && n <= GRP_MAX && q && k && v && o && d_o && lse && dq && dk && dv && delta_ws && N && ld_qkv && ld_o &&
                       ld_do && ld_dqkv, "mtmp_attn_bwd: bad group (n=%d)", n);
    for (int i = 0; i < n; ++i) {
        MTMP_CHECK_ARG(q[i] && k[i] && v[i] && o[i] && d_o[i] && lse[i] && dq[i] && dk[i] && dv[i] && delta_ws[i],
                       "mtmp_attn_bwd: null pointer (stream %d)", i);
        MTMP_CHECK_ARG(!(row_start && row_start[i]) || (kv_len && kv_len[i]), "mtmp_attn_bwd: a packed stream needs kv_len");
        MTMP_CHECK_ARG(attn_shape_ok(B, N[i], H, ld_qkv[i], ld_o[i]) && attn_shape_ok(B, N[i], H, ld_do[i], ld_dqkv[i]),
                       "mtmp_attn_bwd: bad shape B=%d N=%d H=%d", B, N[i], H);
    }
    hipStream_t st = (hipStream_t)stream;
    if (dtype == 0)
        return bwd_entry<float>(n, q, k, v, o, d_o, lse, kv_len, row_start, dq, dk, dv, delta_ws, N, ld_qkv, ld_o, ld_do, ld_dqkv, B, H, scale, st);
    if (dtype == 1)
        return bwd_entry<bf16>(n, q, k, v, o, d_o, lse, kv_len, row_start, dq, dk, dv, delta_ws, N, ld_qkv, ld_o, ld_do, ld_dqkv, B, H, scale, st);
    mtmp_set_error("mtmp_attn_bwd: unknown dtype %d", dtype);
    return MTMP_ERR_ARG;
}

extern "C" int mtmp_attn_bwd(int dtype, const void* q, const void* k, const void* v, const void* o, const void* d_o,
                             const float* lse, const int32_t* kv_len, void* dq, void* dk, void* dv, float* delta_ws,
                             int B, int N, int H, int ld_qkv, int ld_o, int ld_do, int ld_dqkv, float scale,
                             void* stream) {
    return mtmp_attn_bwd_grouped(dtype, 1, &q, &k, &v, &o, &d_o, &lse, &kv_len, nullptr, &dq, &dk, &dv, &delta_ws, &N, &ld_qkv, &ld_o,
                                 &ld_do, &ld_dqkv, B, H, scale, stream);
}

namespace {
template <typename T> struct AttnClsArgs {
    const T* q; const T* k; const T* v; int ld_qkv;
    const T* res; int ld_res;
    T* o_cls; T* r1_cls; float* lse;
    const T* d_o;
    T* dq; T* dk; T* dv; int ld_dqkv;
    const int* kv_len; const int* row_start;
    int B, N, H, cls_tok;
    float scale;
};

template <typename T> MTMP_DEV void load8f(const T* ptr, float (&o)[8]) {
    const f32x4 a = load4<T>(ptr), b = load4<T>(ptr + 4);
    o[0] = a[0]; o[1] = a[1]; o[2] = a[2]; o[3] = a[3]; o[4] = b[0]; o[5] = b[1]; o[6] = b[2]; o[7] = b[3];
}
MTMP_DEV float block_reduce(float v, float* red, bool take_max) {
    v = take_max ? wave_max(v) : wave_sum(v);
    __syncthreads();
    if ((threadIdx.x & 63) == 0) red[threadIdx.x >> 6] = v;
    __syncthreads();
    return take_max ? fmaxf(fmaxf(red[0], red[1]), fmaxf(red[2], red[3])) : (red[0] + red[1]) + (red[2] + red[3]);
}

template <typename T> __global__ __launch_bounds__(256) void attn_cls_fwd_kernel(AttnClsArgs<T> p) {
    extern __shared__ float cls_lds[];
    float* s = cls_lds;
    float* red = s + p.N;
    float* part = red + 4;
    const int b = blockIdx.x / p.H, hd = blockIdx.x % p.H, tid = threadIdx.x;
    const int kv_raw = p.kv_len ? p.kv_len[b] : p.N;
    if (p.row_start && kv_raw <= p.cls_tok) {
        if (tid < DH) {
            const size_t oi = ((size_t)b * p.H + hd) * DH + tid;
            p.o_cls[oi] = from_f32<T>(0.f);
            p.r1_cls[oi] = from_f32<T>(0.f);
            if (tid == 0) p.lse[b * p.H + hd] = 0.f;
        }
        return;
    }
    const bool uniform = kv_raw <= 0;
    const int kvl = uniform ? p.N : min(kv_raw, p.N);
    const size_t row0 = p.row_start ? (size_t)p.row_start[b] : (size_t)b * p.N;
    const T* Kb = p.k + row0 * p.ld_qkv + hd * DH;
    const T* Vb = p.v + row0 * p.ld_qkv + hd * DH;
    const T* qrow = p.q + (row0 + p.cls_tok) * p.ld_qkv + hd * DH;
    const float c2 = uniform ? 0.f : p.scale * LOG2E;
    float q[DH];
#pragma unroll
    for (int c = 0; c < DH / 8; ++c) {
        float t[8];
        load8f<T>(qrow + 8 * c, t);
#pragma unroll
        for (int j = 0; j < 8; ++j) q[8 * c + j] = t[j] * c2;
    }
    float mx = -INFINITY;
    for (int k = tid; k < kvl; k += 256) {
        const T* kr = Kb + (size_t)k * p.ld_qkv;
        float a = 0.f;
#pragma unroll
        for (int c = 0; c < DH / 8; ++c) {
            float t[8];
            load8f<T>(kr + 8 * c, t);
#pragma unroll
            for (int j = 0; j < 8; ++j) a = fmaf(q[8 * c + j], t[j], a);
        }
        s[k] = a;
        mx = fmaxf(mx, a);
    }
    mx = block_reduce(mx, red, true);
    float l = 0.f;
    for (int k = tid; k < kvl; k += 256) {
        const float e = fast_exp2(s[k] - mx);
        s[k] = e;
        l += e;
    }
    l = block_reduce(l, red, false);
    const int dg = tid & 7, kl = tid >> 3;
    float acc[8] = {0.f, 0.f, 0.f, 0.f, 0.f, 0.f, 0.f, 0.f};
    for (int k = kl; k < kvl; k += 32) {
        float t[8];
        load8f<T>(Vb + (size_t)k * p.ld_qkv + 8 * dg, t);
        const float pk = s[k];
#pragma unroll
        for (int j = 0; j < 8; ++j) acc[j] = fmaf(pk, t[j], acc[j]);
    }
#pragma unroll
    for (int j = 0; j < 8; ++j) part[kl * DH + 8 * dg + j] = acc[j];
    __syncthreads();
    if (tid < DH) {
        float o = 0.f;
#pragma unroll 8
        for (int i = 0; i < 32; ++i) o += part[i * DH + tid];
        const T ot = from_f32<T>(o / l);
        const size_t oi = ((size_t)b * p.H + hd) * DH + tid;
        p.o_cls[oi] = ot;
        p.r1_cls[oi] = from_f32<T>(to_f32(ot) + to_f32(p.res[(row0 + p.cls_tok) * p.ld_res + hd * DH + tid]));
        if (tid == 0) p.lse[b * p.H + hd] = mx + log2f(l);
    }
}

template <typename T> MTMP_DEV void store8(T* ptr, const float (&v)[8]) {
    store4<T>(ptr, v[0], v[1], v[2], v[3]);
    store4<T>(ptr + 4, v[4], v[5], v[6], v[7]);
}

template <typename T> __global__ __launch_bounds__(256) void attn_cls_bwd_kernel(AttnClsArgs<T> p) {
    extern __shared__ float cls_lds[];
    float* sP = cls_lds;
    float* sD = sP + p.N;
    float* red = sD + p.N;
    float* part = red + 4;
    const int b = blockIdx.x / p.H, hd = blockIdx.x % p.H, tid = threadIdx.x;
    const int kv_raw = p.kv_len ? p.kv_len[b] : p.N;
    if (p.row_start && kv_raw <= p.cls_tok) return;
    const bool uniform = kv_raw <= 0;
    const int kvl = uniform ? p.N : min(kv_raw, p.N);
    const int nrows = p.row_start ? kvl : p.N;
    const size_t row0 = p.row_start ? (size_t)p.row_start[b] : (size_t)b * p.N;
    const T* Kb = p.k + row0 * p.ld_qkv + hd * DH;
    const T* Vb = p.v + row0 * p.ld_qkv + hd * DH;
    const T* qrow = p.q + (row0 + p.cls_tok) * p.ld_qkv + hd * DH;
    const size_t oi = ((size_t)b * p.H + hd) * DH;
    const float c2 = uniform ? 0.f : p.scale * LOG2E, lse = p.lse[b * p.H + hd];
    float q[DH], g[DH];
    float dl = 0.f;
#pragma unroll
    for (int c = 0; c < DH / 8; ++c) {
        float t[8], d[8], o[8];
        load8f<T>(qrow + 8 * c, t);
        load8f<T>(p.d_o + oi + 8 * c, d);
        load8f<T>(p.o_cls + oi + 8 * c, o);
#pragma unroll
        for (int j = 0; j < 8; ++j) { q[8 * c + j] = t[j] * c2; g[8 * c + j] = d[j]; dl = fmaf(d[j], o[j], dl); }
    }
    for (int k = tid; k < kvl; k += 256) {
        const T* kr = Kb + (size_t)k * p.ld_qkv;
        const T* vr = Vb + (size_t)k * p.ld_qkv;
        float a = 0.f, dp = 0.f;
#pragma unroll
        for (int c = 0; c < DH / 8; ++c) {
            float t[8], u[8];
            load8f<T>(kr + 8 * c, t);
            load8f<T>(vr + 8 * c, u);
#pragma unroll
            for (int j = 0; j < 8; ++j) { a = fmaf(q[8 * c + j], t[j], a); dp = fmaf(g[8 * c + j], u[j], dp); }
        }
        const float pk = fast_exp2(a - lse);
        sP[k] = pk;
        sD[k] = uniform ? 0.f : pk * (dp - dl);
    }
    __syncthreads();
    const int dg = tid & 7, kl = tid >> 3;
    float qd[8], gd[8], zero[8] = {0.f, 0.f, 0.f, 0.f, 0.f, 0.f, 0.f, 0.f}, acc[8] = {0.f, 0.f, 0.f, 0.f, 0.f, 0.f, 0.f, 0.f};
    load8f<T>(qrow + 8 * dg, qd);
    load8f<T>(p.d_o + oi + 8 * dg, gd);
#pragma unroll
    for (int j = 0; j < 8; ++j) qd[j] *= p.scale;
    T* dQb = p.dq + row0 * p.ld_dqkv + hd * DH + 8 * dg;
    T* dKb = p.dk + row0 * p.ld_dqkv + hd * DH + 8 * dg;
    T* dVb = p.dv + row0 * p.ld_dqkv + hd * DH + 8 * dg;
    for (int k = kl; k < nrows; k += 32) {
        const size_t ro = (size_t)k * p.ld_dqkv;
        if (k < kvl) {
            const float ds = sD[k], pk = sP[k];
            float t[8], dk[8], dv[8];
            load8f<T>(Kb + (size_t)k * p.ld_qkv + 8 * dg, t);
#pragma unroll
            for (int j = 0; j < 8; ++j) { acc[j] = fmaf(ds, t[j], acc[j]); dk[j] = ds * qd[j]; dv[j] = pk * gd[j]; }
            store8<T>(dKb + ro, dk);
            store8<T>(dVb + ro, dv);
        } else {
            store8<T>(dKb + ro, zero);
            store8<T>(dVb + ro, zero);
        }
        if (k != p.cls_tok) store8<T>(dQb + ro, zero);
    }
#pragma unroll
    for (int j = 0; j < 8; ++j) part[kl * DH + 8 * dg + j] = acc[j];
    __syncthreads();
    if (tid < DH) {
        float o = 0.f;
#pragma unroll 8
        for (int i = 0; i < 32; ++i) o += part[i * DH + tid];
        p.dq[(row0 + p.cls_tok) * p.ld_dqkv + hd * DH + tid] = from_f32<T>(o * p.scale);
    }
}

bool attn_cls_ok(int B, int N, int H, int cls_tok, int ld) {
    return B > 0 && N > 0 && N <= 8192 && H > 0 && H <= 4 && cls_tok >= 0 && cls_tok < N && ld >= H * DH && ld % 4 == 0;
}
}

extern "C" int mtmp_attn_cls_fwd(int dtype, const void* q, const void* k, const void* v, int ld_qkv, const void* res, int ld_res,
                                 void* o_cls, void* r1_cls, float* lse, const int32_t* kv_len, const int32_t* row_start, int B, int N,
                                 int H, int cls_tok, float scale, void* stream) {
    MTMP_CHECK_ARG(q && k && v && res && o_cls && r1_cls && lse, "mtmp_attn_cls_fwd: null pointer");
    MTMP_CHECK_ARG(attn_cls_ok(B, N, H, cls_tok, ld_qkv) && ld_res >= H * DH && (!row_start || kv_len),
                   "mtmp_attn_cls_fwd: bad argument (B=%d N=%d H=%d cls=%d ld=%d)", B, N, H, cls_tok, ld_qkv);
    const size_t sm = ((size_t)N + 4 + 32 * DH) * sizeof(float);
    hipStream_t st = (hipStream_t)stream;
    if (dtype == 0) {
        AttnClsArgs<float> a{(const float*)q, (const float*)k, (const float*)v, ld_qkv, (const float*)res, ld_res, (float*)o_cls,
                             (float*)r1_cls, lse, nullptr, nullptr, nullptr, nullptr, 0, kv_len, row_start, B, N, H, cls_tok, scale};
        if (int e = set_smem(attn_cls_fwd_kernel<float>, sm)) return e;
        hipLaunchKernelGGL(attn_cls_fwd_kernel<float>, dim3(B * H), dim3(256), sm, st, a);
    } else if (dtype == 1) {
        AttnClsArgs<bf16> a{(const bf16*)q, (const bf16*)k, (const bf16*)v, ld_qkv, (const bf16*)res, ld_res, (bf16*)o_cls,
                            (bf16*)r1_cls, lse, nullptr, nullptr, nullptr, nullptr, 0, kv_len, row_start, B, N, H, cls_tok, scale};
        if (int e = set_smem(attn_cls_fwd_kernel<bf16>, sm)) return e;
        hipLaunchKernelGGL(attn_cls_fwd_kernel<bf16>, dim3(B * H), dim3(256), sm, st, a);
    } else { mtmp_set_error("mtmp_attn_cls_fwd: unknown dtype %d", dtype); return MTMP_ERR_ARG; }
    MTMP_CHECK_LAUNCH("mtmp_attn_cls_fwd");
    return MTMP_OK;
}

extern "C" int mtmp_attn_cls_bwd(int dtype, const void* q, const void* k, const void* v, int ld_qkv, const void* o_cls, const void* d_o,
                                 const float* lse, const int32_t* kv_len, const int32_t* row_start, void* dq, void* dk, void* dv,
                                 int ld_dqkv, int B, int N, int H, int cls_tok, float scale, void* stream) {
    MTMP_CHECK_ARG(q && k && v && o_cls && d_o && lse && dq && dk && dv, "mtmp_attn_cls_bwd: null pointer");
    MTMP_CHECK_ARG(attn_cls_ok(B, N, H, cls_tok, ld_qkv) && ld_dqkv >= H * DH && (!row_start || kv_len),
                   "mtmp_attn_cls_bwd: bad argument (B=%d N=%d H=%d cls=%d ld=%d)", B, N, H, cls_tok, ld_qkv);
    const size_t sm = ((size_t)2 * N + 4 + 32 * DH) * sizeof(float);
    hipStream_t st = (hipStream_t)stream;
    if (dtype == 0) {
        AttnClsArgs<float> a{(const float*)q, (const float*)k, (const float*)v, ld_qkv, nullptr, 0, (float*)o_cls, nullptr,
                             (float*)lse, (const float*)d_o, (float*)dq, (float*)dk, (float*)dv, ld_dqkv, kv_len, row_start, B, N, H,
                             cls_tok, scale};
        if (int e = set_smem(attn_cls_bwd_kernel<float>, sm)) return e;
        hipLaunchKernelGGL(attn_cls_bwd_kernel<float>, dim3(B * H), dim3(256), sm, st, a);
    } else if (dtype == 1) {
        AttnClsArgs<bf16> a{(const bf16*)q, (const bf16*)k, (const bf16*)v, ld_qkv, nullptr, 0, (bf16*)o_cls, nullptr, (float*)lse,
                            (const bf16*)d_o, (bf16*)dq, (bf16*)dk, (bf16*)dv, ld_dqkv, kv_len, row_start, B, N, H, cls_tok, scale};
        if (int e = set_smem(attn_cls_bwd_kernel<bf16>, sm)) return e;
        hipLaunchKernelGGL(attn_cls_bwd_kernel<bf16>, dim3(B * H), dim3(256), sm, st, a);
    } else { mtmp_set_error("mtmp_attn_cls_bwd: unknown dtype %d", dtype); return MTMP_ERR_ARG; }
    MTMP_CHECK_LAUNCH("mtmp_attn_cls_bwd");
    return MTMP_OK;
}

#ifdef MTMP_LAB_CLOCK
extern "C" int mtmp_dbg_read_stamps(long long* host, int n) {
    return (int)hipMemcpyFromSymbol(host, HIP_SYMBOL(mtmp_dbg_stamps), (size_t)n * sizeof(long long));
}
#endif
extern "C" long long mtmp_key_norms_floats(long long rows, int H) { return ((rows + 31) / 32) * H; }

extern "C" int mtmp_key_norms(int dtype, const void* k, float* out, long long rows, int H, int ld, void* stream) {
    MTMP_CHECK_ARG(k && out, "mtmp_key_norms: null pointer");
    MTMP_CHECK_ARG(rows > 0 && rows < (1ll << 31) && H > 0 && H <= 4 && ld >= H * DH && (ld % 8) == 0,
                   "mtmp_key_norms: bad shape rows=%lld H=%d ld=%d", rows, H, ld);
    hipStream_t st = (hipStream_t)stream;
    const int nblk = (int)((rows + 31) / 32);
    if (dtype == 0) hipLaunchKernelGGL(key_norms_kernel<float>, dim3((nblk + 3) / 4), dim3(256), 0, st, (const float*)k, out, (int)rows, H, ld);
    else if (dtype == 1) hipLaunchKernelGGL(key_norms_kernel<bf16>, dim3((nblk + 3) / 4), dim3(256), 0, st, (const bf16*)k, out, (int)rows, H, ld);
    else { mtmp_set_error("mtmp_key_norms: unknown dtype %d", dtype); return MTMP_ERR_ARG; }
    MTMP_CHECK_LAUNCH("mtmp_key_norms");
    return MTMP_OK;
}
```

Measured before the change: 8419 samples/s.

## Make dK/dV backward kernel persistent with cross-item prefetch

Converts the 64-key dK/dV attention backward kernel into a persistent kernel launched with at most one workgroup per CU. Each workgroup loops over work items and prefetches the next item's K/V fragments and its first Q/dO tile while finishing the current one, rotating the LDS stage offset between items. This is meant to cut launch tail and per-workgroup startup latency, at the cost of more register pressure and extra control flow. It also adds a debug hook that can force the kernel form.

Measured after the change: 8422 samples/s (median of 6 runs). Within noise of the previous version (+0.0%).

```diff
diff --git a/include/mtmp.h b/include/mtmp.h
--- a/include/mtmp.h
+++ b/include/mtmp.h
@@ -23,6 +23,7 @@
                           const int32_t* const* row_start, void* const* dq, void* const* dk, void* const* dv,
                           float* const* delta_ws, const int* N, const int* ld_qkv, const int* ld_o, const int* ld_do,
                           const int* ld_dqkv, int B, int H, float scale, void* stream);
+int mtmp_dbg_attn_bwd_form(int form);
 int mtmp_attn_cls_fwd(int dtype, const void* q, const void* k, const void* v, int ld_qkv, const void* res, int ld_res, void* o_cls,
                       void* r1_cls, float* lse, const int32_t* kv_len, const int32_t* row_start, int B, int N, int H, int cls_tok,
                       float scale, void* stream);
diff --git a/medical_tri_modal_pilot_amd/_lib.py b/medical_tri_modal_pilot_amd/_lib.py
--- a/medical_tri_modal_pilot_amd/_lib.py
+++ b/medical_tri_modal_pilot_amd/_lib.py
@@ -15,6 +15,7 @@
     "mtmp_attn_cls_bwd": (c_int, [c_int] + [c_void_p] * 3 + [c_int] + [c_void_p] * 8 + [c_int] * 5 + [c_float, c_void_p]),
     "mtmp_attn_fwd_grouped": (c_int, [c_int, c_int] + [c_void_p] * 13 + [c_int, c_int, c_float, c_void_p]),
     "mtmp_attn_bwd_grouped": (c_int, [c_int, c_int] + [c_void_p] * 17 + [c_int, c_int, c_float, c_void_p]),
+    "mtmp_dbg_attn_bwd_form": (c_int, [c_int]),
     "mtmp_key_norms_floats": (c_longlong, [c_longlong, c_int]),
     "mtmp_key_norms": (c_int, [c_int, c_void_p, c_void_p, c_longlong, c_int, c_int, c_void_p]),
     "mtmp_attn_bwd": (c_int, [c_int] + [c_void_p] * 11 + [c_int] * 7 + [c_float, c_void_p]),
diff --git a/medical_tri_modal_pilot_amd/csrc/attention.hip b/medical_tri_modal_pilot_amd/csrc/attention.hip
--- a/medical_tri_modal_pilot_amd/csrc/attention.hip
+++ b/medical_tri_modal_pilot_amd/csrc/attention.hip
@@ -884,283 +884,338 @@
     return __builtin_bit_cast(unsigned, __builtin_convertvector(f32x2{lo, hi}, bf16x2));
 }
 
+struct RowStream64 {
+    const bf16* base; const bf16* pa;
+    size_t step; int ld, limit, ra, ca, nfull;
+    MTMP_DEV void init(const bf16* src, int ld_, int limit_, int tid) {
+        int rb, cb;
+        DualTile<bf16>::map(tid, ra, rb, ca, cb);
+        base = src; ld = ld_; limit = limit_; nfull = limit_ / KT; step = (size_t)KT * ld_;
+        pa = src + (size_t)ra * ld_ + ca;
+    }
+    MTMP_DEV TileR<bf16> fetch(int t) {
+        TileR<bf16> x;
+        if (t < nfull) {
+            x.a = frag_load<bf16>(pa); x.b = frag_load<bf16>(pa + 32);
+            pa += step;
+        } else {
+            const bf16* row = base + (size_t)min(t * KT + ra, limit - 1) * ld + ca;
+            x.a = frag_load<bf16>(row); x.b = frag_load<bf16>(row + 32);
+        }
+        return x;
+    }
+};
+struct Dkdv64Item { int w, seg, kt, b, hd, kvl, row0, Nq; bool uniform; };
+
 __global__ __launch_bounds__(256, 1) void attn_bwd_dkdv64_kernel(Grouped<AttnBwdArgs<bf16>> grp) {
     using T = bf16;
     using DT = DualTile<T>;
     extern __shared__ __attribute__((aligned(16))) char smem_raw[];
     const int wg = xcd_remap(blockIdx.x, gridDim.x);
-    const int seg = grp_find(grp, wg);
-    const AttnBwdArgs<T>& p = grp.seg[seg];
-    const int w = wg - grp.first[seg];
-    const int nkt = (p.N + DKV64_KEYS - 1) / DKV64_KEYS;
-    const int kt = w % nkt, bh = w / nkt, hd = bh % p.H;
-    const int b = p.row_start ? p.row_start[p.B + 1 + bh / p.H] : bh / p.H;
     const int tid = threadIdx.x, lane = tid & 63, wave = tid >> 6;
     const int r = lane & 31, half = lane >> 5;
-    int kvl = p.kv_len ? min(p.kv_len[b], p.N) : p.N;
-    const int row0 = p.row_start ? p.row_start[b] : b * p.N;
-    const int Nq = p.row_start ? max(kvl, 0) : p.N;
-    if (kt * DKV64_KEYS >= Nq) return;
-    STAMP(0);
-    const bool uniform = kvl <= 0;
-    if (uniform) kvl = Nq;
-    const size_t base = (size_t)row0 * p.ld_qkv + hd * DH;
-    const T* Qb = p.q + base; const T* Kb = p.k + base; const T* Vb = p.v + base;
-    const T* dOb = p.d_o + (size_t)row0 * p.ld_do + hd * DH;
-    const float* Lb = p.lse + ((size_t)b * p.H + hd) * p.N;
-    const float* Db = p.delta + ((size_t)b * p.H + hd) * p.N;
-    const int kw0 = kt * DKV64_KEYS + wave * 64;
-    f32x16 dv00 = {0}, dv01 = {0}, dk00 = {0}, dk01 = {0}, dv10 = {0}, dv11 = {0}, dk10 = {0}, dk11 = {0};
-    if (kt * DKV64_KEYS < kvl) {
-        const float c2 = p.scale * LOG2E;
-        Frag<T> kx[2][4], vx[2][4];
+    const int nitems = grp.first[GRP_MAX];
+    const int lrow = tid & (KT - 1);
+    auto find = [&](int w, Dkdv64Item& x) {
+        for (; w < nitems; w += gridDim.x) {
+            const int seg = grp_find(grp, w);
+            const AttnBwdArgs<T>& p = grp.seg[seg];
+            const int nkt = (p.N + DKV64_KEYS - 1) / DKV64_KEYS;
+            const int i = w - grp.first[seg], kt = i % nkt, bh = i / nkt;
+            const int b = p.row_start ? p.row_start[p.B + 1 + bh / p.H] : bh / p.H;
+            const int kvl = p.kv_len ? min(p.kv_len[b], p.N) : p.N;
+            const int Nq = p.row_start ? max(kvl, 0) : p.N;
+            if (kt * DKV64_KEYS >= Nq) continue;
+            const bool uniform = kvl <= 0;
+            x = Dkdv64Item{w, seg, kt, b, bh % p.H, uniform ? Nq : kvl, p.row_start ? p.row_start[b] : b * p.N, Nq, uniform};
+            return true;
+        }
+        return false;
+    };
+    Frag<T> kx[2][4], vx[2][4];
+    RowStream64 qs, os;
+    TileR<T> qreg, oreg;
+    float lreg = 0.f, dreg = 0.f;
+    auto prefetch = [&](const Dkdv64Item& x) {
+        const AttnBwdArgs<T>& p = grp.seg[x.seg];
+        const size_t base = (size_t)x.row0 * p.ld_qkv + x.hd * DH;
+        const int kw0 = x.kt * DKV64_KEYS + wave * 64;
 #pragma unroll
         for (int kb = 0; kb < 2; ++kb)
 #pragma unroll
             for (int c = 0; c < 4; ++c) {
                 const int key = kw0 + 32 * kb + r;
-                kx[kb][c] = frag_load<T>(Kb + (size_t)min(key, kvl - 1) * p.ld_qkv + 16 * c + 8 * half);
-                vx[kb][c] = frag_load<T>(Vb + (size_t)min(key, kvl - 1) * p.ld_qkv + 16 * c + 8 * half);
-            }
-        const int nq = (Nq + KT - 1) / KT;
-        TileStream<T> qs, os;
-        qs.init(Qb, p.ld_qkv, Nq, tid);
-        os.init(dOb, p.ld_do, Nq, tid);
-        TileR<T> qreg, oreg;
-        const int lrow = tid & (KT - 1);
-        float lreg, dreg;
-        auto stage = [&](int t) { return smem_raw + (t % BWD64_STAGES) * dkdv_stage_bytes<T>(); };
-        auto stage_piece = [&](int k, int tp, int tf) {
-            if (k < 3) {
-                if (tp >= nq) return;
-                char* st_ = stage(tp);
-                if (k == 0) DT::put(st_, qreg, tid);
-                else if (k == 1) DT::put(st_ + DT::BYTES, oreg, tid);
-                else if (tid < KT) {
-                    float* sL = reinterpret_cast<float*>(st_ + 2 * DT::BYTES);
-                    sL[tid] = (tp * KT + tid < Nq) ? -lreg : -INFINITY;
-                    sL[KT + tid] = (tp * KT + tid < Nq) ? -dreg : 0.f;
+                kx[kb][c] = frag_load<T>(p.k + base + (size_t)min(key, x.kvl - 1) * p.ld_qkv + 16 * c + 8 * half);
+                vx[kb][c] = frag_load<T>(p.v + base + (size_t)min(key, x.kvl - 1) * p.ld_qkv + 16 * c + 8 * half);
+            }
+        qs.init(p.q + base, p.ld_qkv, x.Nq, tid);
+        os.init(p.d_o + (size_t)x.row0 * p.ld_do + x.hd * DH, p.ld_do, x.Nq, tid);
+        qreg = qs.fetch(0);
+        oreg = os.fetch(0);
+        const size_t lb = ((size_t)x.b * p.H + x.hd) * p.N + min(lrow, x.Nq - 1);
+        lreg = p.lse[lb];
+        dreg = p.delta[lb];
+    };
+    Dkdv64Item cur;
+    bool have = find(wg, cur);
+    if (have) prefetch(cur);
+    int soff = 0;
+    while (have) {
+        int tid_o = threadIdx.x;
+        asm volatile("" : "+v"(tid_o));
+        const int tid = tid_o, lane = tid & 63, r = lane & 31, half = lane >> 5;
+        const AttnBwdArgs<T>& p = grp.seg[cur.seg];
+        const int kvl = cur.kvl, Nq = cur.Nq, row0 = cur.row0, hd = cur.hd, kt = cur.kt;
+        const bool uniform = cur.uniform;
+        STAMP(0);
+        const float* Lb = p.lse + ((size_t)cur.b * p.H + hd) * p.N;
+        const float* Db = p.delta + ((size_t)cur.b * p.H + hd) * p.N;
+        const int kw0 = kt * DKV64_KEYS + wave * 64;
+        f32x16 dv00 = {0}, dv01 = {0}, dk00 = {0}, dk01 = {0}, dv10 = {0}, dv11 = {0}, dk10 = {0}, dk11 = {0};
+        if (kt * DKV64_KEYS < kvl) {
+            const float c2 = p.scale * LOG2E;
+            const int nq = (Nq + KT - 1) / KT;
+            auto stage = [&](int t) { return smem_raw + ((t + soff) % BWD64_STAGES) * dkdv_stage_bytes<T>(); };
+            auto stage_piece = [&](int k, int tp, int tf) {
+                if (k < 3) {
+                    if (tp >= nq) return;
+                    char* st_ = stage(tp);
+                    if (k == 0) DT::put(st_, qreg, tid);
+                    else if (k == 1) DT::put(st_ + DT::BYTES, oreg, tid);
+                    else if (tid < KT) {
+                        float* sL = reinterpret_cast<float*>(st_ + 2 * DT::BYTES);
+                        sL[tid] = (tp * KT + tid < Nq) ? -lreg : -INFINITY;
+                        sL[KT + tid] = (tp * KT + tid < Nq) ? -dreg : 0.f;
+                    }
+                } else {
+                    if (tf >= nq) return;
+                    if (k == 3) qreg = qs.fetch(tf);
+                    else if (k == 4) oreg = os.fetch(tf);
+                    else {
+                        const int qn = min(tf * KT + lrow, Nq - 1);
+                        lreg = Lb[qn];
+                        dreg = Db[qn];
+                    }
                 }
-            } else {
-                if (tf >= nq) return;
-                if (k == 3) qreg = qs.fetch(tf);
-                else if (k == 4) oreg = os.fetch(tf);
-                else {
-                    const int qn = min(tf * KT + lrow, Nq - 1);
-                    lreg = Lb[qn];
-                    dreg = Db[qn];
+            };
+            auto stage_all = [&](int tp, int tf) {
+#pragma unroll
+                for (int k = 0; k < 6; ++k) stage_piece(k, tp, tf);
+            };
+            bf16x8 kf[2][4], vf[2][4];
+#pragma unroll
+            for (int kb = 0; kb < 2; ++kb)
+#pragma unroll
+                for (int c = 0; c < 4; ++c) {
+                    const bool live = kw0 + 32 * kb + r < kvl;
+                    kf[kb][c] = to_agpr(frag_keep(frag_scale<T>(kx[kb][c], c2), live && !uniform).v);
+                    vf[kb][c] = to_agpr(frag_keep(vx[kb][c], live).v);
                 }
-            }
-        };
-        auto stage_all = [&](int tp, int tf) {
-#pragma unroll
-            for (int k = 0; k < 6; ++k) stage_piece(k, tp, tf);
-        };
-        stage_all(nq, 0);
-        bf16x8 kf[2][4], vf[2][4];
-#pragma unroll
-        for (int kb = 0; kb < 2; ++kb)
-#pragma unroll
-            for (int c = 0; c < 4; ++c) {
-                const bool live = kw0 + 32 * kb + r < kvl;
-                kf[kb][c] = to_agpr(frag_keep(frag_scale<T>(kx[kb][c], c2), live && !uniform).v);
-                vf[kb][c] = to_agpr(frag_keep(vx[kb][c], live).v);
-            }
-        stage_all(0, 1);
-        __syncthreads();
-        const bool active = kw0 < kvl;
-        bf16x8 qa[4], oa[4], tr[2][4];
-        f32x16 cL, cD;
-        struct LaneOffs { unsigned rowE, rowO, cst, trA, trB; };
-        LaneOffs lo;
+            stage_all(0, 1);
+            __syncthreads();
+            const bool active = kw0 < kvl;
+            bf16x8 qa[4], oa[4], tr[2][4];
+            f32x16 cL, cD;
+            struct LaneOffs { unsigned rowE, rowO, cst, trA, trB; };
+            LaneOffs lo;
+            {
+                const int sr = swz23(r), G = lane >> 4, i16 = lane & 15;
+                lo.rowE = DT::off(sr, half);
+                lo.rowO = DT::off(sr, 2 + half);
+                lo.cst = 2 * DT::BYTES + 32 * half;
+                const int trow = 8 * (G >> 1) + (i16 >> 2), tch = 2 * (G & 1) + ((i16 & 3) >> 1);
+                lo.trA = DT::off(trow, tch) + 8 * (i16 & 1);
+                lo.trB = DT::off(trow + 4, tch) + 8 * (i16 & 1);
+                const unsigned lds0 = (unsigned)(size_t)(__attribute__((address_space(3))) char*)smem_raw;
+                lo.rowE += lds0; lo.rowO += lds0; lo.cst += lds0; lo.trA += lds0; lo.trB += lds0;
+            }
+            typedef __attribute__((address_space(3))) const char lds_cchar;
+            auto lds_at = [](unsigned ofs) { return (lds_cchar*)(size_t)ofs; };
+            auto bases = [&](int t) {
+                const unsigned sb = (unsigned)(((t + soff) % BWD64_STAGES) * dkdv_stage_bytes<T>());
+                LaneOffs x{lo.rowE + sb, lo.rowO + sb, lo.cst + sb, lo.trA + sb, lo.trB + sb};
+                asm volatile("" : "+v"(x.rowE), "+v"(x.rowO), "+v"(x.cst), "+v"(x.trA), "+v"(x.trB));
+                return x;
+            };
+            auto load_rows = [&](const LaneOffs& bs, int qb, int c, bool dO) {
+                typedef __attribute__((address_space(3))) const bf16x8 lds_bf16x8;
+                const bf16x8 v = *(lds_bf16x8*)(lds_at((c & 1) ? bs.rowO : bs.rowE) + 512 * (c >> 1) + 4096 * qb + (dO ? DT::BYTES : 0));
+                if (dO) oa[c] = v; else qa[c] = v;
+            };
+            auto load_const = [&](const LaneOffs& bs, int qb, int k4, bool dlt) {
+                typedef __attribute__((address_space(3))) const f32x4 lds_f32x4;
+                const f32x4 v4 = *(lds_f32x4*)(lds_at(bs.cst) + (dlt ? 4 * KT : 0) + 4 * (32 * qb + 16 * (k4 >> 1) + 4 * (k4 & 1)));
+#pragma unroll
+                for (int i = 0; i < 4; ++i) { if (dlt) cD[4 * k4 + i] = v4[i]; else cL[4 * k4 + i] = v4[i]; }
+            };
+            auto load_tr = [&](const LaneOffs& bs, int qb, int s2, int j) {
+                typedef __attribute__((address_space(3))) s16x4 lds_s16x4;
+                const int imm = 4096 * qb + 2048 * s2 + 512 * (j & 1) + (j < 2 ? DT::BYTES : 0);
+                const s16x4 a = __builtin_amdgcn_ds_read_tr16_b64_v4i16((lds_s16x4*)(lds_at(bs.trA) + imm));
+                const s16x4 b4 = __builtin_amdgcn_ds_read_tr16_b64_v4i16((lds_s16x4*)(lds_at(bs.trB) + imm));
+                typedef short s16x8 __attribute__((ext_vector_type(8)));
+                tr[s2][j] = __builtin_bit_cast(bf16x8, s16x8{a[0], a[1], a[2], a[3], b4[0], b4[1], b4[2], b4[3]});
+            };
+            auto slot = [&](auto mode_tag, f32x16& sN, f32x16& dN, const bf16x8 (&kfb)[4], const bf16x8 (&vfb)[4], f32x16& sC, f32x16& dC,
+                            PackedUnit& out, const PackedUnit& in, f32x16& dv0, f32x16& dv1, f32x16& dk0, f32x16& dk1,
+                            const LaneOffs& st_rows, int qb_rows, const LaneOffs& st_tr, int qb_tr, int tp, int tf) {
+                constexpr int MODE = decltype(mode_tag)::value;
+#pragma unroll
+                for (int i = 0; i < 16; ++i) {
+                    if (i == 0) MTMP_MFMA_FIRST(sN, qa[0], kfb[0], cL);
+                    else if (i < 4) MTMP_MFMA_NEXT(sN, qa[i], kfb[i]);
+                    else if (i == 4) MTMP_MFMA_FIRST(dN, oa[0], vfb[0], cD);
+                    else if (i < 8) MTMP_MFMA_NEXT(dN, oa[i - 4], vfb[i - 4]);
+                    else {
+                        const int s2 = (i - 8) >> 2, j = (i - 8) & 3;
+                        if (j == 0) MTMP_MFMA_ACC(dv0, tr[s2][0], in.p[s2]);
+                        else if (j == 1) MTMP_MFMA_ACC(dv1, tr[s2][1], in.p[s2]);
+                        else if (j == 2) MTMP_MFMA_ACC(dk0, tr[s2][2], in.d[s2]);
+                        else MTMP_MFMA_ACC(dk1, tr[s2][3], in.d[s2]);
+                    }
+                    const float e = fast_exp2(sC[i]);
+                    if (i > 0) dC[i - 1] *= sC[i - 1];
+                    sC[i] = e;
+                    if (i & 1) out.p[i >> 3][(i & 7) >> 1] = cvt_pk_bf16(sC[i - 1], e);
+                    if (i >= 2 && !(i & 1)) out.d[(i - 2) >> 3][((i - 2) & 7) >> 1] = cvt_pk_bf16(dC[i - 2], dC[i - 1]);
+                    if (i == 15) {
+                        dC[15] *= e;
+                        out.d[1][3] = cvt_pk_bf16(dC[14], dC[15]);
+                    }
+                    if (MODE == 1) {
+                        if (i < 4) load_rows(st_rows, qb_rows, i, false);
+                        else if (i < 8) load_rows(st_rows, qb_rows, i - 4, true);
+                        else load_tr(st_tr, qb_tr, (i - 8) >> 2, (i - 8) & 3);
+                        if (i >= 1 && i < 5) load_const(st_rows, qb_rows, i - 1, false);
+                        else if (i >= 5 && i < 9) load_const(st_rows, qb_rows, i - 5, true);
+                    }
+                    if (MODE == 2 && (i & 1) && i < 12) stage_piece(i >> 1, tp, tf);
+                    __builtin_amdgcn_sched_barrier(0);
+                }
+            };
+            f32x16 sA, dA, sB, dB;
+            PackedUnit fX, fY;
+#pragma unroll
+            for (int t = 0; t < 16; ++t) { sB[t] = -INFINITY; dB[t] = 0.f; }
+#pragma unroll
+            for (int s2 = 0; s2 < 2; ++s2) {
+                fX.p[s2] = u32x4_t{0, 0, 0, 0}; fX.d[s2] = u32x4_t{0, 0, 0, 0};
+#pragma unroll
+                for (int j = 0; j < 4; ++j) tr[s2][j] = frag_zero<T>().v;
+            }
+            if (active) {
+                const LaneOffs b0 = bases(0);
+#pragma unroll
+                for (int c = 0; c < 4; ++c) {
+                    load_rows(b0, 0, c, false); load_rows(b0, 0, c, true);
+                    load_const(b0, 0, c, false); load_const(b0, 0, c, true);
+                }
+            }
+            const std::integral_constant<int, 0> plain{};
+            const std::integral_constant<int, 1> loads{};
+            const std::integral_constant<int, 2> staging{};
+            STAMP(1);
+            for (int it = 0; it < nq; ++it) {
+                STAMP(2 + 8 * it);
+                const LaneOffs cur = bases(it);
+                const LaneOffs nxt = bases(it + 1 < nq ? it + 1 : it);
+                if (active) {
+                    __builtin_amdgcn_sched_barrier(0);
+                    STAMP(3 + 8 * it);
+                    slot(staging, sA, dA, kf[0], vf[0], sB, dB, fY, fX, dv00, dv01, dk00, dk01, cur, 0, cur, 0, it + 1, it + 2);
+                    STAMP(4 + 8 * it);
+                    slot(loads, sB, dB, kf[1], vf[1], sA, dA, fX, fY, dv10, dv11, dk10, dk11, cur, 1, cur, 0, 0, 0);
+                    STAMP(5 + 8 * it);
+                    slot(plain, sA, dA, kf[0], vf[0], sB, dB, fY, fX, dv00, dv01, dk00, dk01, cur, 0, cur, 0, 0, 0);
+                    STAMP(6 + 8 * it);
+                } else {
+                    stage_all(it + 1, it + 2);
+                }
+                __syncthreads();
+                if (active) {
+                    STAMP(7 + 8 * it);
+                    slot(loads, sB, dB, kf[1], vf[1], sA, dA, fX, fY, dv10, dv11, dk10, dk11, nxt, 0, cur, 1, 0, 0);
+                    STAMP(8 + 8 * it);
+                }
+            }
+            if (active) {
+#pragma unroll
+                for (int i = 0; i < 16; ++i) {
+                    if (i < 8) {
+                        const int s2 = i >> 2, j = i & 3;
+                        if (j == 0) MTMP_MFMA_ACC(dv00, tr[s2][0], fX.p[s2]);
+                        else if (j == 1) MTMP_MFMA_ACC(dv01, tr[s2][1], fX.p[s2]);
+                        else if (j == 2) MTMP_MFMA_ACC(dk00, tr[s2][2], fX.d[s2]);
+                        else MTMP_MFMA_ACC(dk01, tr[s2][3], fX.d[s2]);
+                    }
+                    const float e = fast_exp2(sB[i]);
+                    dB[i] *= e;
+                    sB[i] = e;
+                    if (i & 1) {
+                        fY.p[i >> 3][(i & 7) >> 1] = cvt_pk_bf16(sB[i - 1], e);
+                        fY.d[i >> 3][(i & 7) >> 1] = cvt_pk_bf16(dB[i - 1], dB[i]);
+                    }
+                    __builtin_amdgcn_sched_barrier(0);
+                }
+#pragma unroll
+                for (int s2 = 0; s2 < 2; ++s2) {
+                    MTMP_MFMA_ACC(dv10, tr[s2][0], fY.p[s2]);
+                    MTMP_MFMA_ACC(dv11, tr[s2][1], fY.p[s2]);
+                    MTMP_MFMA_ACC(dk10, tr[s2][2], fY.d[s2]);
+                    MTMP_MFMA_ACC(dk11, tr[s2][3], fY.d[s2]);
+                }
+            }
+            STAMP(150);
+            asm volatile("s_nop 15\n\ts_nop 15" : "+a"(dv00), "+a"(dv01), "+a"(dk00), "+a"(dk01), "+a"(dv10), "+a"(dv11), "+a"(dk10), "+a"(dk11));
+            soff = (soff + nq) % BWD64_STAGES;
+        }
+        have = find(cur.w + gridDim.x, cur);
+        if (have) prefetch(cur);
+        else {
+#pragma unroll
+            for (int kb = 0; kb < 2; ++kb)
+#pragma unroll
+                for (int c = 0; c < 4; ++c) { kx[kb][c] = frag_zero<T>(); vx[kb][c] = frag_zero<T>(); }
+        }
+        T* sOut = reinterpret_cast<T*>(smem_raw + BWD64_STAGES * dkdv_stage_bytes<T>() + wave * DKV64_OUT_BYTES);
+#pragma unroll
+        for (int kb = 0; kb < 2; ++kb) {
+            const int key = kw0 + 32 * kb + r;
+            const bool live = key < kvl;
+            const bool wk = live && !uniform;
+#pragma unroll
+            for (int dt = 0; dt < 2; ++dt)
+#pragma unroll
+                for (int g = 0; g < 4; ++g) {
+                    const f32x16& ak = kb ? (dt ? dk11 : dk10) : (dt ? dk01 : dk00);
+                    const f32x16& av = kb ? (dt ? dv11 : dv10) : (dt ? dv01 : dv00);
+                    const int d0 = 32 * dt + 8 * g + 4 * half;
+                    store4<T>(sOut + (32 * kb + r) * LDT + d0, wk ? ak[4 * g] * p.scale : 0.f, wk ? ak[4 * g + 1] * p.scale : 0.f,
+                              wk ? ak[4 * g + 2] * p.scale : 0.f, wk ? ak[4 * g + 3] * p.scale : 0.f);
+                    store4<T>(sOut + (64 + 32 * kb + r) * LDT + d0, live ? av[4 * g] : 0.f, live ? av[4 * g + 1] : 0.f,
+                              live ? av[4 * g + 2] : 0.f, live ? av[4 * g + 3] : 0.f);
+                }
+        }
+        asm volatile("s_waitcnt lgkmcnt(0)" ::: "memory");
         {
-            const int sr = swz23(r), G = lane >> 4, i16 = lane & 15;
-            lo.rowE = DT::off(sr, half);
-            lo.rowO = DT::off(sr, 2 + half);
-            lo.cst = 2 * DT::BYTES + 32 * half;
-            const int trow = 8 * (G >> 1) + (i16 >> 2), tch = 2 * (G & 1) + ((i16 & 3) >> 1);
-            lo.trA = DT::off(trow, tch) + 8 * (i16 & 1);
-            lo.trB = DT::off(trow + 4, tch) + 8 * (i16 & 1);
-            const unsigned lds0 = (unsigned)(size_t)(__attribute__((address_space(3))) char*)smem_raw;
-            lo.rowE += lds0; lo.rowO += lds0; lo.cst += lds0; lo.trA += lds0; lo.trB += lds0;
-        }
-        typedef __attribute__((address_space(3))) const char lds_cchar;
-        auto lds_at = [](unsigned ofs) { return (lds_cchar*)(size_t)ofs; };
-        auto bases = [&](int t) {
-            const unsigned sb = (unsigned)((t % BWD64_STAGES) * dkdv_stage_bytes<T>());
-            LaneOffs x{lo.rowE + sb, lo.rowO + sb, lo.cst + sb, lo.trA + sb, lo.trB + sb};
-            asm volatile("" : "+v"(x.rowE), "+v"(x.rowO), "+v"(x.cst), "+v"(x.trA), "+v"(x.trB));
-            return x;
-        };
-        auto load_rows = [&](const LaneOffs& bs, int qb, int c, bool dO) {
-            typedef __attribute__((address_space(3))) const bf16x8 lds_bf16x8;
-            const bf16x8 v = *(lds_bf16x8*)(lds_at((c & 1) ? bs.rowO : bs.rowE) + 512 * (c >> 1) + 4096 * qb + (dO ? DT::BYTES : 0));
-            if (dO) oa[c] = v; else qa[c] = v;
-        };
-        auto load_const = [&](const LaneOffs& bs, int qb, int k4, bool dlt) {
-            typedef __attribute__((address_space(3))) const f32x4 lds_f32x4;
-            const f32x4 v4 = *(lds_f32x4*)(lds_at(bs.cst) + (dlt ? 4 * KT : 0) + 4 * (32 * qb + 16 * (k4 >> 1) + 4 * (k4 & 1)));
-#pragma unroll
-            for (int i = 0; i < 4; ++i) { if (dlt) cD[4 * k4 + i] = v4[i]; else cL[4 * k4 + i] = v4[i]; }
-        };
-        auto load_tr = [&](const LaneOffs& bs, int qb, int s2, int j) {
-            typedef __attribute__((address_space(3))) s16x4 lds_s16x4;
-            const int imm = 4096 * qb + 2048 * s2 + 512 * (j & 1) + (j < 2 ? DT::BYTES : 0);
-            const s16x4 a = __builtin_amdgcn_ds_read_tr16_b64_v4i16((lds_s16x4*)(lds_at(bs.trA) + imm));
-            const s16x4 b4 = __builtin_amdgcn_ds_read_tr16_b64_v4i16((lds_s16x4*)(lds_at(bs.trB) + imm));
-            typedef short s16x8 __attribute__((ext_vector_type(8)));
-            tr[s2][j] = __builtin_bit_cast(bf16x8, s16x8{a[0], a[1], a[2], a[3], b4[0], b4[1], b4[2], b4[3]});
-        };
-        auto slot = [&](auto mode_tag, f32x16& sN, f32x16& dN, const bf16x8 (&kfb)[4], const bf16x8 (&vfb)[4], f32x16& sC, f32x16& dC,
-                        PackedUnit& out, const PackedUnit& in, f32x16& dv0, f32x16& dv1, f32x16& dk0, f32x16& dk1,
-                        const LaneOffs& st_rows, int qb_rows, const LaneOffs& st_tr, int qb_tr, int tp, int tf) {
-            constexpr int MODE = decltype(mode_tag)::value;
-#pragma unroll
-            for (int i = 0; i < 16; ++i) {
-                if (i == 0) MTMP_MFMA_FIRST(sN, qa[0], kfb[0], cL);
-                else if (i < 4) MTMP_MFMA_NEXT(sN, qa[i], kfb[i]);
-                else if (i == 4) MTMP_MFMA_FIRST(dN, oa[0], vfb[0], cD);
-                else if (i < 8) MTMP_MFMA_NEXT(dN, oa[i - 4], vfb[i - 4]);
-                else {
-                    const int s2 = (i - 8) >> 2, j = (i - 8) & 3;
-                    if (j == 0) MTMP_MFMA_ACC(dv0, tr[s2][0], in.p[s2]);
-                    else if (j == 1) MTMP_MFMA_ACC(dv1, tr[s2][1], in.p[s2]);
-                    else if (j == 2) MTMP_MFMA_ACC(dk0, tr[s2][2], in.d[s2]);
-                    else MTMP_MFMA_ACC(dk1, tr[s2][3], in.d[s2]);
+            const int rsub = lane >> 3, ch = lane & 7;
+            u32x4_t ok[8], ov[8];
+#pragma unroll
+            for (int ps = 0; ps < 8; ++ps) {
+                ok[ps] = *reinterpret_cast<const u32x4_t*>(reinterpret_cast<const char*>(sOut + (8 * ps + rsub) * LDT) + 16 * ch);
+                ov[ps] = *reinterpret_cast<const u32x4_t*>(reinterpret_cast<const char*>(sOut + (64 + 8 * ps + rsub) * LDT) + 16 * ch);
+            }
+            T* krow = p.dk + ((size_t)row0 + kw0 + rsub) * p.ld_dqkv + hd * DH + 8 * ch;
+            T* vrow = p.dv + ((size_t)row0 + kw0 + rsub) * p.ld_dqkv + hd * DH + 8 * ch;
+#pragma unroll
+            for (int ps = 0; ps < 8; ++ps)
+                if (kw0 + 8 * ps + rsub < Nq) {
+                    *reinterpret_cast<u32x4_t*>(krow + (size_t)8 * ps * p.ld_dqkv) = ok[ps];
+                    *reinterpret_cast<u32x4_t*>(vrow + (size_t)8 * ps * p.ld_dqkv) = ov[ps];
                 }
-                const float e = fast_exp2(sC[i]);
-                if (i > 0) dC[i - 1] *= sC[i - 1];
-                sC[i] = e;
-                if (i & 1) out.p[i >> 3][(i & 7) >> 1] = cvt_pk_bf16(sC[i - 1], e);
-                if (i >= 2 && !(i & 1)) out.d[(i - 2) >> 3][((i - 2) & 7) >> 1] = cvt_pk_bf16(dC[i - 2], dC[i - 1]);
-                if (i == 15) {
-                    dC[15] *= e;
-                    out.d[1][3] = cvt_pk_bf16(dC[14], dC[15]);
-                }
-                if (MODE == 1) {
-                    if (i < 4) load_rows(st_rows, qb_rows, i, false);
-                    else if (i < 8) load_rows(st_rows, qb_rows, i - 4, true);
-                    else load_tr(st_tr, qb_tr, (i - 8) >> 2, (i - 8) & 3);
-                    if (i >= 1 && i < 5) load_const(st_rows, qb_rows, i - 1, false);
-                    else if (i >= 5 && i < 9) load_const(st_rows, qb_rows, i - 5, true);
-                }
-                if (MODE == 2 && (i & 1) && i < 12) stage_piece(i >> 1, tp, tf);
-                __builtin_amdgcn_sched_barrier(0);
-            }
-        };
-        f32x16 sA, dA, sB, dB;
-        PackedUnit fX, fY;
-#pragma unroll
-        for (int t = 0; t < 16; ++t) { sB[t] = -INFINITY; dB[t] = 0.f; }
-#pragma unroll
-        for (int s2 = 0; s2 < 2; ++s2) {
-            fX.p[s2] = u32x4_t{0, 0, 0, 0}; fX.d[s2] = u32x4_t{0, 0, 0, 0};
-#pragma unroll
-            for (int j = 0; j < 4; ++j) tr[s2][j] = frag_zero<T>().v;
-        }
-        if (active) {
-            const LaneOffs b0 = bases(0);
-#pragma unroll
-            for (int c = 0; c < 4; ++c) {
-                load_rows(b0, 0, c, false); load_rows(b0, 0, c, true);
-                load_const(b0, 0, c, false); load_const(b0, 0, c, true);
-            }
-        }
-        const std::integral_constant<int, 0> plain{};
-        const std::integral_constant<int, 1> loads{};
-        const std::integral_constant<int, 2> staging{};
-        STAMP(1);
-        for (int it = 0; it < nq; ++it) {
-            STAMP(2 + 8 * it);
-            const LaneOffs cur = bases(it);
-            const LaneOffs nxt = bases(it + 1 < nq ? it + 1 : it);
-            if (active) {
-                __builtin_amdgcn_sched_barrier(0);
-                STAMP(3 + 8 * it);
-                slot(staging, sA, dA, kf[0], vf[0], sB, dB, fY, fX, dv00, dv01, dk00, dk01, cur, 0, cur, 0, it + 1, it + 2);
-                STAMP(4 + 8 * it);
-                slot(loads, sB, dB, kf[1], vf[1], sA, dA, fX, fY, dv10, dv11, dk10, dk11, cur, 1, cur, 0, 0, 0);
-                STAMP(5 + 8 * it);
-                slot(plain, sA, dA, kf[0], vf[0], sB, dB, fY, fX, dv00, dv01, dk00, dk01, cur, 0, cur, 0, 0, 0);
-                STAMP(6 + 8 * it);
-            } else {
-                stage_all(it + 1, it + 2);
-            }
-            __syncthreads();
-            if (active) {
-                STAMP(7 + 8 * it);
-                slot(loads, sB, dB, kf[1], vf[1], sA, dA, fX, fY, dv10, dv11, dk10, dk11, nxt, 0, cur, 1, 0, 0);
-                STAMP(8 + 8 * it);
-            }
-        }
-        if (active) {
-#pragma unroll
-            for (int i = 0; i < 16; ++i) {
-                if (i < 8) {
-                    const int s2 = i >> 2, j = i & 3;
-                    if (j == 0) MTMP_MFMA_ACC(dv00, tr[s2][0], fX.p[s2]);
-                    else if (j == 1) MTMP_MFMA_ACC(dv01, tr[s2][1], fX.p[s2]);
-                    else if (j == 2) MTMP_MFMA_ACC(dk00, tr[s2][2], fX.d[s2]);
-                    else MTMP_MFMA_ACC(dk01, tr[s2][3], fX.d[s2]);
-                }
-                const float e = fast_exp2(sB[i]);
-                dB[i] *= e;
-                sB[i] = e;
-                if (i & 1) {
-                    fY.p[i >> 3][(i & 7) >> 1] = cvt_pk_bf16(sB[i - 1], e);
-                    fY.d[i >> 3][(i & 7) >> 1] = cvt_pk_bf16(dB[i - 1], dB[i]);
-                }
-                __builtin_amdgcn_sched_barrier(0);
-            }
-#pragma unroll
-            for (int s2 = 0; s2 < 2; ++s2) {
-                MTMP_MFMA_ACC(dv10, tr[s2][0], fY.p[s2]);
-                MTMP_MFMA_ACC(dv11, tr[s2][1], fY.p[s2]);
-                MTMP_MFMA_ACC(dk10, tr[s2][2], fY.d[s2]);
-                MTMP_MFMA_ACC(dk11, tr[s2][3], fY.d[s2]);
-            }
-        }
-        STAMP(150);
-        asm volatile("s_nop 15\n\ts_nop 15" : "+a"(dv00), "+a"(dv01), "+a"(dk00), "+a"(dk01), "+a"(dv10), "+a"(dv11), "+a"(dk10), "+a"(dk11));
-    }
-    T* sOut = reinterpret_cast<T*>(smem_raw + BWD64_STAGES * dkdv_stage_bytes<T>() + wave * DKV64_OUT_BYTES);
-#pragma unroll
-    for (int kb = 0; kb < 2; ++kb) {
-        const int key = kw0 + 32 * kb + r;
-        const bool live = key < kvl;
-        const bool wk = live && !uniform;
-#pragma unroll
-        for (int dt = 0; dt < 2; ++dt)
-#pragma unroll
-            for (int g = 0; g < 4; ++g) {
-                const f32x16& ak = kb ? (dt ? dk11 : dk10) : (dt ? dk01 : dk00);
-                const f32x16& av = kb ? (dt ? dv11 : dv10) : (dt ? dv01 : dv00);
-                const int d0 = 32 * dt + 8 * g + 4 * half;
-                store4<T>(sOut + (32 * kb + r) * LDT + d0, wk ? ak[4 * g] * p.scale : 0.f, wk ? ak[4 * g + 1] * p.scale : 0.f,
-                          wk ? ak[4 * g + 2] * p.scale : 0.f, wk ? ak[4 * g + 3] * p.scale : 0.f);
-                store4<T>(sOut + (64 + 32 * kb + r) * LDT + d0, live ? av[4 * g] : 0.f, live ? av[4 * g + 1] : 0.f,
-                          live ? av[4 * g + 2] : 0.f, live ? av[4 * g + 3] : 0.f);
-            }
-    }
-    asm volatile("s_waitcnt lgkmcnt(0)" ::: "memory");
-    {
-        const int rsub = lane >> 3, ch = lane & 7;
-        u32x4_t ok[8], ov[8];
-#pragma unroll
-        for (int ps = 0; ps < 8; ++ps) {
-            ok[ps] = *reinterpret_cast<const u32x4_t*>(reinterpret_cast<const char*>(sOut + (8 * ps + rsub) * LDT) + 16 * ch);
-            ov[ps] = *reinterpret_cast<const u32x4_t*>(reinterpret_cast<const char*>(sOut + (64 + 8 * ps + rsub) * LDT) + 16 * ch);
-        }
-        T* krow = p.dk + ((size_t)row0 + kw0 + rsub) * p.ld_dqkv + hd * DH + 8 * ch;
-        T* vrow = p.dv + ((size_t)row0 + kw0 + rsub) * p.ld_dqkv + hd * DH + 8 * ch;
-#pragma unroll
-        for (int ps = 0; ps < 8; ++ps)
-            if (kw0 + 8 * ps + rsub < Nq) {
-                *reinterpret_cast<u32x4_t*>(krow + (size_t)8 * ps * p.ld_dqkv) = ok[ps];
-                *reinterpret_cast<u32x4_t*>(vrow + (size_t)8 * ps * p.ld_dqkv) = ov[ps];
-            }
-    }
-    STAMP(151);
+        }
+        STAMP(151);
+    }
 }
 
 template <typename T> size_t fwd_smem() { return (size_t)2 * fwd_stage_elems<T>() * sizeof(T); }
@@ -1199,6 +1254,20 @@
     MTMP_CHECK_LAUNCH("mtmp_attn_fwd");
     return MTMP_OK;
 }
+
+int cu_count() {
+    static int n = 0;
+    if (n == 0) {
+        int dev = 0, v = 0;
+        if (hipGetDevice(&dev) == hipSuccess && hipDeviceGetAttribute(&v, hipDeviceAttributeMultiprocessorCount, dev) == hipSuccess && v > 0)
+            n = v;
+        else
+            return 256;
+    }
+    return n;
+}
+
+int g_bwd_form = 0;
 
 template <typename T> int launch_bwd(int n, const AttnBwdArgs<T>* segs, hipStream_t st) {
     int nwg;
@@ -1209,13 +1278,13 @@
     if constexpr (sizeof(T) == 2) {
         int nmax = 0;
         for (int i = 0; i < n; ++i) nmax = segs[i].N > nmax ? segs[i].N : nmax;
-        if (nmax >= BWD64_MIN_ROWS) {
-            int nwg64;
+        if (g_bwd_form == 2 || (g_bwd_form == 0 && nmax >= BWD64_MIN_ROWS)) {
+            int items;
             const Grouped<AttnBwdArgs<T>> g64 =
-                make_group(n, segs, [](const AttnBwdArgs<T>& a) { return ((a.N + DKV64_KEYS - 1) / DKV64_KEYS) * a.H * a.B; }, nwg64);
+                make_group(n, segs, [](const AttnBwdArgs<T>& a) { return ((a.N + DKV64_KEYS - 1) / DKV64_KEYS) * a.H * a.B; }, items);
             const size_t sm64 = (size_t)BWD64_STAGES * dkdv_stage_bytes<T>() + 4 * DKV64_OUT_BYTES;
             if (int e = set_smem(attn_bwd_dkdv64_kernel, sm64)) return e;
-            hipLaunchKernelGGL(attn_bwd_dkdv64_kernel, dim3(nwg64), dim3(256), sm64, st, g64);
+            hipLaunchKernelGGL(attn_bwd_dkdv64_kernel, dim3(items < cu_count() ? items : cu_count()), dim3(256), sm64, st, g64);
             MTMP_CHECK_LAUNCH("mtmp_attn_bwd(dkdv64)");
             return MTMP_OK;
         }
@@ -1305,6 +1374,12 @@
         return bwd_entry<bf16>(n, q, k, v, o, d_o, lse, kv_len, row_start, dq, dk, dv, delta_ws, N, ld_qkv, ld_o, ld_do, ld_dqkv, B, H, scale, st);
     mtmp_set_error("mtmp_attn_bwd: unknown dtype %d", dtype);
     return MTMP_ERR_ARG;
+}
+
+extern "C" int mtmp_dbg_attn_bwd_form(int form) {
+    MTMP_CHECK_ARG(form >= 0 && form <= 2, "mtmp_dbg_attn_bwd_form: bad form %d", form);
+    g_bwd_form = form;
+    return MTMP_OK;
 }
 
 extern "C" int mtmp_attn_bwd(int dtype, const void* q, const void* k, const void* v, const void* o, const void* d_o,
```
